# kluonj/HelFEM

Measured on AMD Instinct MI355X. Metric: scf_iteration_wall_time_fock_plus_geneig_nbf4230, lower is better.
Workload: dtype f64; 1 GPU; diatomic Z1=7 Z2=7 R=2.068 PBE, nelem=5 nnodes=15 nquad=75 lmmax=[20,20] (Nbf=4230, Nang=61, Nrad=70), XC grid 92x13, symmetry blocks [1380, 1470, 1380]: J+XC Fock build + eig_gsym_sub + density per step; parallelism=shard1, density=occupied orbitals of the core Hamiltonian

## Files before the change

helfem_amd/csrc/hip/common.h:

```cpp
#pragma once
#include <hip/hip_runtime.h>
#include <cstdint>
#include <cstring>
#include <map>
#include <stdexcept>
#include <string>
#include <vector>

#include "../../../include/helfem_gpu.h"
#include "../host/atomic_basis.h"
#include "../host/diatomic_basis.h"
#include "../host/tuning.h"

namespace hfg {
using helfem::TrdMode, helfem::tuning;

void set_error(const std::string &msg);

#define HFG_HIP_CHECK(expr)                                                                          \
  do {                                                                                               \
    hipError_t _e = (expr);                                                                          \
    if (_e != hipSuccess)                                                                            \
      throw std::runtime_error(std::string("HIP error: ") + hipGetErrorString(_e) + " in " + #expr + \
                               " (" + __FILE__ + ":" + std::to_string(__LINE__) + ")");              \
  } while (0)

template <typename T>
struct DevBuf {
  T *p = nullptr;
  size_t n = 0;
  DevBuf() {}
  DevBuf(const DevBuf &) = delete;
  DevBuf &operator=(const DevBuf &) = delete;
  ~DevBuf() { release(); }
  void release() {
    if (p) (void)hipFree(p);
    p = nullptr;
    n = 0;
  }
  void resize(size_t count) {
    if (count <= n) return;
    release();
    HFG_HIP_CHECK(hipMalloc((void **)&p, count * sizeof(T)));
    n = count;
  }
  void upload(const std::vector<T> &h, hipStream_t s) {
    resize(h.size() ? h.size() : 1);
    if (h.size()) HFG_HIP_CHECK(hipMemcpyAsync(p, h.data(), h.size() * sizeof(T), hipMemcpyHostToDevice, s));
  }
};

template <typename T>
bool upload_cached(DevBuf<T> &buf, std::vector<T> &cache, const std::vector<T> &h, hipStream_t s) {
  if (buf.p && cache.size() == h.size() && buf.n >= h.size() &&
      (h.empty() || memcmp((const void *)cache.data(), (const void *)h.data(), h.size() * sizeof(T)) == 0))
    return false;
  HFG_HIP_CHECK(hipStreamSynchronize(s));
  cache = h;
  buf.upload(cache, s);
  return true;
}

struct ProfEntry {
  double ms = 0.0;
  int64_t launches = 0;
  std::vector<std::pair<hipEvent_t, hipEvent_t> > pending;
};

}

struct hfg_dev_tables;

struct hfg_ctx {
  int device = 0;
  hipStream_t stream = nullptr;
  bool own_stream = false;
  hipStream_t side_stream = nullptr;
  hipEvent_t side_ev[2] = {nullptr, nullptr};
  hipStream_t side();
  bool avoid_side = false;
  void drop_side();
  int shard_rank = 0, shard_n = 1;
  const double *fixed_sinvh = nullptr;
  unsigned long fixed_gen = 0;
  void fix_sinvh(const double *p) {
    fixed_sinvh = p;
    fixed_gen++;
  }
  bool profiling = false;
  std::map<std::string, hfg::ProfEntry> prof;
  std::vector<hipEvent_t> event_pool;
  hfg::DevBuf<double> ws[8];
  hfg::DevBuf<double> hstage;
  double *pinned = nullptr;
  size_t pinned_bytes = 0;

  void *pinned_buf(size_t bytes);
  hipEvent_t get_event();
  void prof_begin(const char *name);
  void prof_end(const char *name);
  void prof_collect();
};

struct hfg_basis {
  int kind = 0;
  helfem::diatomic::TwoDBasis b;
  helfem::atomic::TwoDBasis ab;
  hfg_dev_tables *dev = nullptr;
  hfg_dev_tables *dev_rs = nullptr;
  int dev_device = -1;
  hfg::DevBuf<double> dev_tei;
  bool tei_on_device = false;

  size_t Nbf() const { return kind ? ab.Nbf() : b.Nbf(); }
  size_t Ndummy() const { return kind ? ab.Nbf() : b.Ndummy(); }
  size_t Nrad() const { return kind ? ab.Nrad() : b.Nrad(); }
  size_t Nang() const { return kind ? ab.Nang() : b.Nang(); }
  size_t Nel() const { return kind ? ab.Nel() : b.Nel(); }
  size_t max_Nprim() const { return kind ? ab.max_Nprim() : b.max_Nprim(); }
  bool have_tei() const { return tei_on_device || (kind ? ab.have_tei : b.have_tei); }
};

namespace hfg {
struct GemmTask {
  const double *A;
  const double *B;
  double *C;
  int M, N, K, lda, ldb, ldc;
  int tA = 0, tB = 0;
  double alpha = 1.0, beta = 0.0;
  int sym = 0;
  int over = 0;
};
static_assert(sizeof(GemmTask) == 80, "GemmTask is compared bytewise: keep it free of padding");

struct ProfScope {
  hfg_ctx *c;
  const char *n;
  ProfScope(hfg_ctx *ctx, const char *name) : c(ctx), n(name) {
    if (c->profiling) c->prof_begin(n);
  }
  ~ProfScope() {
    if (c->profiling) c->prof_end(n);
  }
};
}
```

helfem_amd/csrc/hip/dc.hip:

```cpp
#include "common.h"
#include <cstring>
#include "wave.h"

namespace hfg {

constexpr int DC_LEAF = 16;
constexpr int DC_MAXB = 8;
#define DC_EPS 2.220446049250313e-16

struct DCNode {
  int blk, lo, mid, hi;
};

struct DCBatch {
  int n[DC_MAXB];
  double *d[DC_MAXB];
  double *d2[DC_MAXB];
  double *e[DC_MAXB];
  double *Qa[DC_MAXB], *Qb[DC_MAXB];
  double *U[DC_MAXB], *Qg[DC_MAXB], *Qn[DC_MAXB];
  double *Ds[DC_MAXB], *zs[DC_MAXB], *dnd[DC_MAXB], *znd[DC_MAXB], *mu[DC_MAXB], *lam[DC_MAXB], *zhat[DC_MAXB];
  double *rotc[DC_MAXB], *rots[DC_MAXB];
  int *src[DC_MAXB], *flag[DC_MAXB], *nd[DC_MAXB], *org[DC_MAXB], *roti[DC_MAXB], *rotj[DC_MAXB], *rank[DC_MAXB];
  int *ndpos[DC_MAXB];
};

__global__ void k_dc_tear(DCBatch b, const DCNode *__restrict__ nodes, int nnodes, double *__restrict__ rho) {
  int i = blockIdx.x * blockDim.x + threadIdx.x;
  if (i >= nnodes) return;
  DCNode nd = nodes[i];
  double r = b.e[nd.blk][nd.mid - 1];
  rho[i] = r;
  b.d[nd.blk][nd.mid - 1] -= fabs(r);
  b.d[nd.blk][nd.mid] -= fabs(r);
}

__global__ __launch_bounds__(64) void k_dc_leaf(DCBatch b, const DCNode *__restrict__ leaves, int nleaves,
                                                int *__restrict__ status) {
  __shared__ double ds[DC_LEAF], es[DC_LEAF], zt[DC_LEAF][DC_LEAF + 1];
  int li = blockIdx.x;
  if (li >= nleaves) return;
  DCNode lf = leaves[li];
  const int lo = lf.lo, s = lf.hi - lf.lo;
  const int lane = threadIdx.x;
  const int ld = b.n[lf.blk];
  double *d = b.d[lf.blk], *e = b.e[lf.blk];
  if (lane < s) {
    ds[lane] = d[lo + lane];
    es[lane] = (lane < s - 1) ? e[lo + lane] : 0.0;
    for (int c = 0; c < s; c++) zt[c][lane] = (c == lane) ? 1.0 : 0.0;
  }
  __syncthreads();
  for (int l = 0; l < s; l++) {
    int iter = 0;
    int m;
    do {
      for (m = l; m + 1 < s; m++) {
        double dd = fabs(ds[m]) + fabs(ds[m + 1]);
        if (fabs(es[m]) <= DC_EPS * dd) break;
      }
      if (m != l) {
        if (iter++ == 300) {
          if (lane == 0) status[0] = 1;
          break;
        }
        double g = (ds[l + 1] - ds[l]) / (2.0 * es[l]);
        double r = hypot(g, 1.0);
        g = ds[m] - ds[l] + es[l] / (g + (g >= 0.0 ? fabs(r) : -fabs(r)));
        double sn = 1.0, c = 1.0, p = 0.0;
        bool under = false;
        for (int i = m - 1; i >= l; i--) {
          double f = sn * es[i], bb = c * es[i];
          r = hypot(f, g);
          __syncthreads();
          es[i + 1] = r;
          if (r == 0.0) {
            ds[i + 1] -= p;
            es[m] = 0.0;
            under = true;
            __syncthreads();
            break;
          }
          sn = f / r;
          c = g / r;
          g = ds[i + 1] - p;
          r = (ds[i] - g) * sn + 2.0 * c * bb;
          p = sn * r;
          __syncthreads();
          ds[i + 1] = g + p;
          g = c * r - bb;
          if (lane < s) {
            double fz = zt[i + 1][lane], zi = zt[i][lane];
            zt[i + 1][lane] = sn * zi + c * fz;
            zt[i][lane] = c * zi - sn * fz;
          }
          __syncthreads();
        }
        if (under) continue;
        __syncthreads();
        ds[l] -= p;
        es[l] = g;
        es[m] = 0.0;
        __syncthreads();
      }
    } while (m != l);
  }
  __syncthreads();
  if (lane < s) {
    double v = ds[lane];
    int rk = 0;
    for (int j = 0; j < s; j++) rk += (ds[j] < v) || (ds[j] == v && j < lane);
    d[lo + rk] = v;
    double *Q = b.Qa[lf.blk];
    for (int k = 0; k < s; k++) Q[(size_t)(lo + rk) * ld + lo + k] = zt[lane][k];
  }
}

constexpr int DC_SQZ = 20;
__global__ __launch_bounds__(256) void k_dc_prepare(DCBatch b, const DCNode *__restrict__ nodes,
                                                    const double *__restrict__ rho_all, int node0,
                                                    int *__restrict__ kcount, int *__restrict__ nrot,
                                                    double *__restrict__ rho_eff, GemmTask *__restrict__ tasks,
                                                    double *__restrict__ gscratch, size_t gstride) {
  extern __shared__ double lds_[];
  double *sh = gscratch ? gscratch + (size_t)blockIdx.x * gstride : lds_;
  const int ni = node0 + blockIdx.x;
  const DCNode nd = nodes[ni];
  const int blk = nd.blk, lo = nd.lo, mid = nd.mid, hi = nd.hi;
  const int n1 = mid - lo, n = hi - lo;
  const int ld = b.n[blk];
  double *sD = sh;
  double *sz = sh + n;
  int *ssrc = (int *)(sh + 2 * n);
  int *sflag = ssrc + n;
  int *snd = sflag + n;
  int *rm = snd + n;
  unsigned long long *rotw = (unsigned long long *)(rm + n);
  __shared__ int nrm_sh, candk_sh;
  __shared__ double red[8];
  __shared__ double tol_sh;
  __shared__ int k_sh;
  const double *d = b.d[blk];
  const double *Q = b.Qa[blk];
  const double rs = rho_all[ni];
  const double sgn = (rs >= 0.0) ? 1.0 : -1.0;
  const double rho = 2.0 * fabs(rs);
  const double isq2 = 0.7071067811865475244;

  double dmax = 0.0, zmax = 0.0;
  for (int j = threadIdx.x; j < n; j += blockDim.x) {
    double Dj = d[lo + j];
    double zj = (j < n1 ? Q[(size_t)(lo + j) * ld + (mid - 1)] : sgn * Q[(size_t)(lo + j) * ld + mid]) * isq2;
    int pos;
    if (j < n1) {
      int a = 0, c = n - n1;
      while (a < c) {
        int h = (a + c) >> 1;
        if (d[mid + h] < Dj) a = h + 1;
        else c = h;
      }
      pos = j + a;
    } else {
      int a = 0, c = n1;
      while (a < c) {
        int h = (a + c) >> 1;
        if (d[lo + h] <= Dj) a = h + 1;
        else c = h;
      }
      pos = (j - n1) + a;
    }
    sD[pos] = Dj;
    sz[pos] = zj;
    ssrc[pos] = j;
    dmax = fmax(dmax, fabs(Dj));
    zmax = fmax(zmax, fabs(zj));
  }
  double m2 = fmax(dmax, zmax);
  m2 = wave_max(m2);
  zmax = wave_max(zmax);
  if ((threadIdx.x & 63) == 0) {
    red[threadIdx.x >> 6] = m2;
    red[4 + (threadIdx.x >> 6)] = zmax;
  }
  __syncthreads();
  const double mm = fmax(fmax(red[0], red[1]), fmax(red[2], red[3]));
  const double zz = fmax(fmax(red[4], red[5]), fmax(red[6], red[7]));
  const double tol = 8.0 * DC_EPS * mm;
  __shared__ int scan[256];
  int fast = 0, fast_k = 0;
  if (!(rho * zz <= tol)) {
    const int tid = threadIdx.x;
    const int chunk = (n + 255) / 256, c0 = tid * chunk, c1 = min(n, c0 + chunk);
    int cnt = 0;
    for (int j = c0; j < c1; j++) {
      const int small = (rho * fabs(sz[j]) <= tol) ? 1 : 0;
      sflag[j] = small;
      cnt += 1 - small;
    }
    scan[tid] = cnt;
    __syncthreads();
    for (int off = 1; off < 256; off <<= 1) {
      const int v = (tid >= off) ? scan[tid - off] : 0;
      __syncthreads();
      scan[tid] += v;
      __syncthreads();
    }
    fast_k = scan[255];
    int r = scan[tid] - cnt;
    for (int j = c0; j < c1; j++)
      if (!sflag[j]) snd[r++] = j;
    __syncthreads();
    int rot = 0;
    for (int base = 0; base < fast_k; base += 256) {
      const int q = base + tid;
      int f = 0;
      if (q >= 1 && q < fast_k) {
        const int pj = snd[q - 1], j = snd[q];
        const double zj = sz[j], zp = sz[pj], t = sD[j] - sD[pj];
        f = (fabs(t * zj * zp) <= tol * (zj * zj + zp * zp)) ? 1 : 0;
      }
      const unsigned long long m = __ballot(f);
      if ((tid & 63) == 0) rotw[(base >> 6) + (tid >> 6)] = m;
      rot |= f;
    }
    fast = __syncthreads_or(rot) ? 0 : 1;
  }
  if (threadIdx.x == 0) {
    nrm_sh = 0;
    candk_sh = fast_k;
  }
  if (threadIdx.x == 0) {
    tol_sh = tol;
    int k = 0, nr = 0;
    int *ndl = snd;
    int *ri = b.roti[blk] + lo, *rj = b.rotj[blk] + lo;
    double *rc = b.rotc[blk] + lo, *rsn = b.rots[blk] + lo;
    if (rho * zz <= tol) {
      for (int j = 0; j < n; j++) sflag[j] = 1;
    } else if (fast) {
      k = fast_k;
    } else if (n <= 256 * DC_SQZ) {
      const int K = fast_k, nw = (K + 63) >> 6;
      int q = 1;
      while (q < K) {
        int wq = q >> 6;
        unsigned long long m = rotw[wq] & (~0ull << (q & 63));
        while (m == 0 && ++wq < nw) m = rotw[wq];
        if (m == 0) break;
        q = (wq << 6) + __ffsll((long long)m) - 1;
        if (q >= K) break;
        int pq = q - 1, pj = snd[pq];
        double zp = sz[pj], dp = sD[pj];
        while (q < K) {
          const int j = snd[q];
          const double zj = sz[j], dj = sD[j], t = dj - dp;
          if (!(fabs(t * zj * zp) <= tol * (zj * zj + zp * zp))) {
            q++;
            break;
          }
          const double tau = hypot(zj, zp);
          const double c = zj / tau, sn = -zp / tau;
          sz[j] = tau;
          sz[pj] = 0.0;
          ri[nr] = pj;
          rj[nr] = j;
          rc[nr] = c;
          rsn[nr] = sn;
          rm[nr] = pq;
          nr++;
          const double tt = dp * c * c + dj * sn * sn;
          const double dn = dp * sn * sn + dj * c * c;
          sD[j] = dn;
          sD[pj] = tt;
          sflag[pj] = 1;
          pj = j;
          pq = q;
          zp = tau;
          dp = dn;
          q++;
        }
      }
      k = K - nr;
      nrm_sh = nr;
    } else {
      int pj = -1;
      double zp = 0.0, dp = 0.0;
      for (int j = 0; j < n; j++) {
        const double zj = sz[j], dj = sD[j];
        if (rho * fabs(zj) <= tol) {
          sflag[j] = 1;
          continue;
        }
        sflag[j] = 0;
        if (pj < 0) {
          pj = j;
          zp = zj;
          dp = dj;
          continue;
        }
        const double t = dj - dp;
        if (fabs(t * zj * zp) <= tol * (zj * zj + zp * zp)) {
          const double tau = hypot(zj, zp);
          const double c = zj / tau, s = -zp / tau;
          sz[j] = tau;
          sz[pj] = 0.0;
          ri[nr] = pj;
          rj[nr] = j;
          rc[nr] = c;
          rsn[nr] = s;
          nr++;
          const double tt = dp * c * c + dj * s * s;
          const double dn = dp * s * s + dj * c * c;
          sD[j] = dn;
          sD[pj] = tt;
          sflag[pj] = 1;
          pj = j;
          zp = tau;
          dp = dn;
        } else {
          ndl[k++] = pj;
          pj = j;
          zp = zj;
          dp = dj;
        }
      }
      if (pj >= 0) ndl[k++] = pj;
    }
    k_sh = k;
    kcount[ni] = k;
    nrot[ni] = nr;
    rho_eff[ni] = rho;
    GemmTask t;
    t.A = b.Qg[blk] + (size_t)lo * ld + lo;
    t.B = b.U[blk] + (size_t)lo * ld + lo;
    t.C = b.Qn[blk] + (size_t)lo * ld + lo;
    t.M = n;
    t.N = k;
    t.K = k;
    t.lda = t.ldb = t.ldc = ld;
    tasks[blockIdx.x] = t;
  }
  __syncthreads();
  if (nrm_sh > 0) {
    const int K = candk_sh, nrm = nrm_sh;
    const int chunk = (K + 255) / 256, c0 = threadIdx.x * chunk;
    int vals[DC_SQZ], newi[DC_SQZ];
#pragma unroll
    for (int e = 0; e < DC_SQZ; e++) {
      const int q = c0 + e;
      newi[e] = -1;
      vals[e] = 0;
      if (e < chunk && q < K) {
        int a = 0, c = nrm;
        while (a < c) {
          const int h = (a + c) >> 1;
          if (rm[h] < q) a = h + 1;
          else c = h;
        }
        if (!(a < nrm && rm[a] == q)) {
          newi[e] = q - a;
          vals[e] = snd[q];
        }
      }
    }
    __syncthreads();
#pragma unroll
    for (int e = 0; e < DC_SQZ; e++)
      if (newi[e] >= 0) snd[newi[e]] = vals[e];
    __syncthreads();
  }
  const int k = k_sh;
  for (int j = threadIdx.x; j < n; j += blockDim.x) {
    b.Ds[blk][lo + j] = sD[j];
    b.zs[blk][lo + j] = sz[j];
    b.src[blk][lo + j] = ssrc[j];
    b.flag[blk][lo + j] = sflag[j];
  }
  for (int c = threadIdx.x; c < k; c += blockDim.x) {
    int sidx = snd[c];
    b.ndpos[blk][lo + sidx] = c;
    b.nd[blk][lo + c] = sidx;
    b.dnd[blk][lo + c] = sD[sidx];
    b.znd[blk][lo + c] = sz[sidx];
  }
}

__global__ __launch_bounds__(256) void k_dc_rotate(DCBatch b, const DCNode *__restrict__ nodes, int node0,
                                                   const int *__restrict__ nrot) {
  const int ni = node0 + blockIdx.y;
  const DCNode nd = nodes[ni];
  const int nr = nrot[ni];
  if (nr == 0) return;
  const int lo = nd.lo, n = nd.hi - nd.lo, blk = nd.blk;
  const int ld = b.n[blk];
  const int r = blockIdx.x * blockDim.x + threadIdx.x;
  __shared__ int scp[256], scj[256];
  __shared__ double sc[256], ss[256];
  const int *src = b.src[blk] + lo;
  double *Q = b.Qa[blk] + lo + r;
  for (int t0 = 0; t0 < nr; t0 += 256) {
    const int t = t0 + threadIdx.x;
    if (t < nr) {
      scp[threadIdx.x] = lo + src[b.roti[blk][lo + t]];
      scj[threadIdx.x] = lo + src[b.rotj[blk][lo + t]];
      sc[threadIdx.x] = b.rotc[blk][lo + t];
      ss[threadIdx.x] = b.rots[blk][lo + t];
    }
    __syncthreads();
    if (r < n) {
      const int cnt = min(256, nr - t0);
      for (int u = 0; u < cnt; u++) {
        const int cp = scp[u], cj = scj[u];
        const double c = sc[u], s = ss[u];
        const double qp = Q[(size_t)cp * ld], qj = Q[(size_t)cj * ld];
        Q[(size_t)cp * ld] = c * qp + s * qj;
        Q[(size_t)cj * ld] = -s * qp + c * qj;
      }
    }
    __syncthreads();
  }
}


__global__ __launch_bounds__(256) void k_dc_secular(DCBatch b, const DCNode *__restrict__ nodes, int node0,
                                                    const int *__restrict__ kcount,
                                                    const double *__restrict__ rho_eff) {
  const int ni = node0 + blockIdx.y;
  const int k = kcount[ni];
  const int i = blockIdx.x * 4 + (threadIdx.x >> 6);
  if (i >= k) return;
  const int lane = threadIdx.x & 63;
  const DCNode nd = nodes[ni];
  const int blk = nd.blk, lo = nd.lo;
  const double *d = b.dnd[blk] + lo, *z = b.znd[blk] + lo;
  const double rho = rho_eff[ni];
  int org;
  double lob, hib, y;
  if (i < k - 1) {
    double gap = d[i + 1] - d[i];
    double midp = 0.5 * gap;
    double di = d[i];
    double s = 0.0;
    for (int j = lane; j < k; j += 64) s += z[j] * z[j] / ((d[j] - di) - midp);
    double fm = 1.0 + rho * wave_sum(s);
    if (fm > 0.0) {
      org = i;
      lob = 0.0;
      hib = midp;
    } else {
      org = i + 1;
      lob = -midp;
      hib = 0.0;
    }
  } else {
    org = k - 1;
    double s = 0.0;
    for (int j = lane; j < k; j += 64) s += z[j] * z[j];
    lob = 0.0;
    hib = rho * wave_sum(s);
  }
  const double dorg = d[org];
  y = 0.5 * (lob + hib);
  for (int it = 0; it < 100; it++) {
    double psi = 0.0, phi = 0.0, dpsi = 0.0, dphi = 0.0;
    for (int j = lane; j < k; j += 64) {
      double D = (d[j] - dorg) - y;
      double t = z[j] * z[j] / D;
      if (j <= i) {
        psi += t;
        dpsi += t / D;
      } else {
        phi += t;
        dphi += t / D;
      }
    }
    psi = rho * wave_sum(psi);
    phi = rho * wave_sum(phi);
    dpsi = rho * wave_sum(dpsi);
    dphi = rho * wave_sum(dphi);
    double w = 1.0 + psi + phi;
    double err = 16.0 * DC_EPS * (1.0 + fabs(psi) + fabs(phi)) + DC_EPS * fabs(y) * (dpsi + dphi);
    if (fabs(w) <= err) break;
    if (w < 0.0) lob = y;
    else hib = y;
    double eta;
    if (i < k - 1) {
      double Di = (d[i] - dorg) - y, Dq = (d[i + 1] - dorg) - y;
      double c = w - Di * dpsi - Dq * dphi;
      double a = (Di + Dq) * w - Di * Dq * (dpsi + dphi);
      double bb = Di * Dq * w;
      if (c == 0.0) eta = (a != 0.0) ? bb / a : 0.0;
      else {
        double disc = a * a - 4.0 * bb * c;
        disc = sqrt(fmax(disc, 0.0));
        eta = (a <= 0.0) ? (a - disc) / (2.0 * c) : 2.0 * bb / (a + disc);
      }
    } else {
      double Di = -y;
      double c = w - Di * dpsi;
      double S = Di * Di * dpsi;
      eta = (c != 0.0) ? Di + S / c : 0.0;
    }
    double yn = y + eta;
    if (!(yn > lob && yn < hib)) yn = 0.5 * (lob + hib);
    bool done = (yn == y) || (hib - lob <= 2.0 * DC_EPS * fmax(fabs(lob), fabs(hib)));
    y = yn;
    if (done) break;
  }
  if (lane == 0) {
    b.org[blk][lo + i] = org;
    b.mu[blk][lo + i] = y;
    b.lam[blk][lo + i] = dorg + y;
  }
}

__global__ __launch_bounds__(256) void k_dc_zhat(DCBatch b, const DCNode *__restrict__ nodes, int node0,
                                                 const int *__restrict__ kcount, const double *__restrict__ rho_eff) {
  const int ni = node0 + blockIdx.y;
  const int k = kcount[ni];
  const int j = blockIdx.x * 4 + (threadIdx.x >> 6);
  if (j >= k) return;
  const int lane = threadIdx.x & 63;
  const DCNode nd = nodes[ni];
  const int blk = nd.blk, lo = nd.lo;
  const double *d = b.dnd[blk] + lo, *mu = b.mu[blk] + lo;
  const int *org = b.org[blk] + lo;
  const double dj = d[j];
  double prod = 1.0;
  for (int i = lane; i < k; i += 64) {
    double num = (d[org[i]] - dj) + mu[i];
    prod *= (i == j) ? num : num / (d[i] - dj);
  }
  prod = wave_prod(prod);
  if (lane == 0) {
    double zh = sqrt(fabs(prod) / rho_eff[ni]);
    b.zhat[blk][lo + j] = (b.znd[blk][lo + j] >= 0.0) ? zh : -zh;
  }
}

__global__ __launch_bounds__(256) void k_dc_U(DCBatch b, const DCNode *__restrict__ nodes, int node0,
                                              const int *__restrict__ kcount) {
  const int ni = node0 + blockIdx.y;
  const int k = kcount[ni];
  const int i = blockIdx.x * 4 + (threadIdx.x >> 6);
  if (i >= k) return;
  const int lane = threadIdx.x & 63;
  const DCNode nd = nodes[ni];
  const int blk = nd.blk, lo = nd.lo;
  const int ld = b.n[blk];
  const double *d = b.dnd[blk] + lo, *zh = b.zhat[blk] + lo;
  const double dorg = d[b.org[blk][lo + i]], mui = b.mu[blk][lo + i];
  double s = 0.0;
  for (int j = lane; j < k; j += 64) {
    double v = zh[j] / ((d[j] - dorg) - mui);
    s += v * v;
  }
  s = 1.0 / sqrt(wave_sum(s));
  double *Ucol = b.U[blk] + (size_t)(lo + i) * ld + lo;
  for (int j = lane; j < k; j += 64) Ucol[j] = zh[j] / ((d[j] - dorg) - mui) * s;
}

__global__ void k_dc_gather(DCBatch b, const DCNode *__restrict__ nodes, int node0,
                            const int *__restrict__ kcount) {
  const int ni = node0 + blockIdx.z;
  const int k = kcount[ni];
  const int c = blockIdx.y;
  if (c >= k) return;
  const DCNode nd = nodes[ni];
  const int blk = nd.blk, lo = nd.lo, n = nd.hi - nd.lo;
  const int ld = b.n[blk];
  int r = blockIdx.x * blockDim.x + threadIdx.x;
  if (r >= n) return;
  const double *Q = b.Qa[blk];
  int sidx = b.nd[blk][lo + c];
  int col = lo + b.src[blk][lo + sidx];
  b.Qg[blk][(size_t)(lo + c) * ld + lo + r] = Q[(size_t)col * ld + lo + r];
}

__global__ __launch_bounds__(256) void k_dc_rank(DCBatch b, const DCNode *__restrict__ nodes, int node0,
                                                 const int *__restrict__ kcount) {
  extern __shared__ double sh[];
  const int ni = node0 + blockIdx.x;
  const DCNode nd = nodes[ni];
  const int blk = nd.blk, lo = nd.lo, n = nd.hi - nd.lo;
  if ((int)blockIdx.y * 32 >= n) return;
  const int *flag = b.flag[blk] + lo;
  for (int s = threadIdx.x; s < n; s += blockDim.x) {
    sh[s] = flag[s] ? b.Ds[blk][lo + s] : b.lam[blk][lo + b.ndpos[blk][lo + s]];
  }
  __syncthreads();
  const int s = blockIdx.y * 32 + (threadIdx.x >> 3), part = threadIdx.x & 7;
  const int per = (n + 7) >> 3, j0 = part * per, j1 = min(n, j0 + per);
  const bool ok = s < n;
  const double v = ok ? sh[s] : 0.0;
  int rk = 0;
  if (ok) {
    int j = j0;
    for (; j + 8 <= j1; j += 8) {
#pragma unroll
      for (int u = 0; u < 8; u++) {
        const double x = sh[j + u];
        rk += (x < v) || (x == v && j + u < s);
      }
    }
    for (; j < j1; j++) {
      const double x = sh[j];
      rk += (x < v) || (x == v && j < s);
    }
  }
  rk += __builtin_amdgcn_update_dpp(0, rk, 0xb1, 0xf, 0xf, true);
  rk += __builtin_amdgcn_update_dpp(0, rk, 0x4e, 0xf, 0xf, true);
  rk += __builtin_amdgcn_update_dpp(0, rk, 0x141, 0xf, 0xf, true);
  if (ok && part == 0) {
    b.rank[blk][lo + s] = rk;
    b.d2[blk][lo + rk] = v;
  }
}

__global__ void k_dc_scatter(DCBatch b, const DCNode *__restrict__ nodes, int node0, const int *__restrict__ kcount) {
  const int ni = node0 + blockIdx.z;
  const DCNode nd = nodes[ni];
  const int blk = nd.blk, lo = nd.lo, n = nd.hi - nd.lo;
  const int s = blockIdx.y;
  if (s >= n) return;
  int r = blockIdx.x * blockDim.x + threadIdx.x;
  if (r >= n) return;
  const int ld = b.n[blk];
  const int k = kcount[ni];
  const double *Q = b.Qa[blk];
  int rk = b.rank[blk][lo + s];
  double v;
  if (b.flag[blk][lo + s]) {
    v = Q[(size_t)(lo + b.src[blk][lo + s]) * ld + lo + r];
  } else {
    const int *ndl = b.nd[blk] + lo;
    int a = 0, c = k;
    while (a < c) {
      int h = (a + c) >> 1;
      if (ndl[h] < s) a = h + 1;
      else c = h;
    }
    v = b.Qn[blk][(size_t)(lo + a) * ld + lo + r];
  }
  b.Qb[blk][(size_t)(lo + rk) * ld + lo + r] = v;
}

__global__ void k_dc_copyback(DCBatch b, const DCNode *__restrict__ nodes, int node0) {
  const int ni = node0 + blockIdx.z;
  const DCNode nd = nodes[ni];
  const int blk = nd.blk, lo = nd.lo, n = nd.hi - nd.lo;
  const int c = blockIdx.y;
  if (c >= n) return;
  int r = blockIdx.x * blockDim.x + threadIdx.x;
  if (r >= n) return;
  const int ld = b.n[blk];
  b.Qa[blk][(size_t)(lo + c) * ld + lo + r] = b.Qb[blk][(size_t)(lo + c) * ld + lo + r];
  if (c == 0) b.d[blk][lo + r] = b.d2[blk][lo + r];
}

void gemm_tasklist64_dev(hfg_ctx *ctx, const GemmTask *dtasks, int ntasks, int maxM, int maxN);
typedef double double4_t __attribute__((ext_vector_type(4)));

__global__ __launch_bounds__(256) void k_dgemm_tasks(const GemmTask *__restrict__ tasks) {
  constexpr int BM = 64, BN = 64, BK = 16, PAD = 16;
  __shared__ double As[BK][BM + PAD];
  __shared__ double Bs[BK][BN + PAD];
  const GemmTask t = tasks[blockIdx.y];
  const int M = t.M, N = t.N, K = t.K;
  if (M <= 0 || N <= 0) return;
  const int nbm = (M + BM - 1) / BM, nbn = (N + BN - 1) / BN;
  if ((int)blockIdx.x >= nbm * nbn) return;
  const int bm = (blockIdx.x % nbm) * BM, bn = (blockIdx.x / nbm) * BN;
  const int tid = threadIdx.x, wave = tid >> 6, lane = tid & 63;
  const int wm = (wave & 1) * 32, wn = (wave >> 1) * 32;
  const int l15 = lane & 15, l4 = lane >> 4;
  double4_t acc[2][2];
  for (int i = 0; i < 2; i++)
    for (int j = 0; j < 2; j++) acc[i][j] = (double4_t){0.0, 0.0, 0.0, 0.0};
  for (int k0 = 0; k0 < K; k0 += BK) {
    __syncthreads();
#pragma unroll
    for (int r = 0; r < 4; r++) {
      int e = tid + 256 * r;
      int m = e % BM, kk = e / BM;
      int gm = bm + m, gk = k0 + kk;
      As[kk][m] = (gm < M && gk < K) ? t.A[(size_t)gk * t.lda + gm] : 0.0;
      int k2 = e % BK, n2 = e / BK;
      int gn = bn + n2, gk2 = k0 + k2;
      Bs[k2][n2] = (gn < N && gk2 < K) ? t.B[(size_t)gn * t.ldb + gk2] : 0.0;
    }
    __syncthreads();
#pragma unroll
    for (int kk = 0; kk < BK; kk += 4) {
      double fa[2], fb[2];
      for (int i = 0; i < 2; i++) fa[i] = As[kk + l4][wm + i * 16 + l15];
      for (int j = 0; j < 2; j++) fb[j] = Bs[kk + l4][wn + j * 16 + l15];
      for (int i = 0; i < 2; i++)
        for (int j = 0; j < 2; j++) acc[i][j] = __builtin_amdgcn_mfma_f64_16x16x4f64(fb[j], fa[i], acc[i][j], 0, 0, 0);
    }
  }
  for (int i = 0; i < 2; i++)
    for (int j = 0; j < 2; j++)
      for (int r = 0; r < 4; r++) {
        int gm = bm + wm + i * 16 + l15, gn = bn + wn + j * 16 + l4 + 4 * r;
        if (gm < M && gn < N) t.C[(size_t)gn * t.ldc + gm] = acc[i][j][r];
      }
}

void gemm_tasks_dev(hfg_ctx *ctx, const GemmTask *dtasks, int ntasks, int max_tiles) {
  if (ntasks <= 0 || max_tiles <= 0) return;
  for (int t0 = 0; t0 < ntasks; t0 += 65535) {
    int nt = std::min(65535, ntasks - t0);
    hipLaunchKernelGGL(k_dgemm_tasks, dim3(max_tiles, nt), dim3(256), 0, ctx->stream, dtasks + t0);
  }
  HFG_HIP_CHECK(hipGetLastError());
}

struct DCWork {
  DevBuf<double> prep_scratch;
  DevBuf<double> d2[DC_MAXB], Qb[DC_MAXB], U[DC_MAXB], Qg[DC_MAXB], Qn[DC_MAXB];
  DevBuf<double> vec[DC_MAXB];
  DevBuf<int> ivec[DC_MAXB];
  DevBuf<DCNode> nodes;
  DevBuf<double> rho, rho_eff;
  DevBuf<int> kcount, nrot, status;
  DevBuf<GemmTask> tasks;
  std::vector<int> key;
  std::vector<DCNode> hnodes;
  std::vector<int> level_off;
  std::vector<int> level_maxn;
  int nleaves = 0;
};
static std::map<hfg_ctx *, DCWork *> g_dc;
void dc_release(hfg_ctx *ctx) {
  auto it = g_dc.find(ctx);
  if (it != g_dc.end()) {
    delete it->second;
    g_dc.erase(it);
  }
}

static int build_tree(int blk, int lo, int hi, std::vector<std::vector<DCNode> > &byheight) {
  DCNode nd;
  nd.blk = blk;
  nd.lo = lo;
  nd.hi = hi;
  if (hi - lo <= DC_LEAF) {
    nd.mid = lo;
    if (byheight.empty()) byheight.resize(1);
    byheight[0].push_back(nd);
    return 0;
  }
  int mid = lo + (hi - lo) / 2;
  nd.mid = mid;
  int h = 1 + std::max(build_tree(blk, lo, mid, byheight), build_tree(blk, mid, hi, byheight));
  if ((int)byheight.size() <= h) byheight.resize(h + 1);
  byheight[h].push_back(nd);
  return h;
}

void tridiag_dc_batch(hfg_ctx *ctx, int nblk, const int *ns, double *const *d, double *const *e, double *const *Z) {
  if (nblk > DC_MAXB) throw std::logic_error("tridiag_dc_batch: too many blocks");
  DCWork *wp;
  auto it = g_dc.find(ctx);
  if (it == g_dc.end()) {
    wp = new DCWork();
    g_dc[ctx] = wp;
  } else
    wp = it->second;
  DCWork &w = *wp;
  hipStream_t s = ctx->stream;
  std::vector<int> key(ns, ns + nblk);
  if (key != w.key) {
    std::vector<std::vector<DCNode> > byh;
    for (int b = 0; b < nblk; b++) build_tree(b, 0, ns[b], byh);
    w.hnodes.clear();
    w.level_off.clear();
    w.level_maxn.clear();
    w.hnodes.insert(w.hnodes.end(), byh[0].begin(), byh[0].end());
    w.nleaves = (int)byh[0].size();
    for (size_t h = 1; h < byh.size(); h++) {
      w.level_off.push_back((int)w.hnodes.size());
      int mx = 0;
      for (auto &nd : byh[h]) mx = std::max(mx, nd.hi - nd.lo);
      w.level_maxn.push_back(mx);
      w.hnodes.insert(w.hnodes.end(), byh[h].begin(), byh[h].end());
    }
    w.level_off.push_back((int)w.hnodes.size());
    w.nodes.resize(w.hnodes.size());
    HFG_HIP_CHECK(hipMemcpyAsync(w.nodes.p, w.hnodes.data(), sizeof(DCNode) * w.hnodes.size(), hipMemcpyHostToDevice, s));
    HFG_HIP_CHECK(hipStreamSynchronize(s));
    w.key = key;
    w.rho.resize(w.hnodes.size());
    w.rho_eff.resize(w.hnodes.size());
    w.kcount.resize(w.hnodes.size());
    w.nrot.resize(w.hnodes.size());
    w.tasks.resize(w.hnodes.size());
    w.status.resize(4);
  }
  DCBatch b;
  int nmax = 0;
  for (int i = 0; i < nblk; i++) {
    int n = ns[i];
    nmax = std::max(nmax, n);
    size_t nn = (size_t)n * n;
    w.d2[i].resize(n);
    w.Qb[i].resize(nn);
    w.U[i].resize(nn);
    w.Qg[i].resize(nn);
    w.Qn[i].resize(nn);
    w.vec[i].resize((size_t)9 * n);
    w.ivec[i].resize((size_t)8 * n);
    b.n[i] = n;
    b.d[i] = d[i];
    b.d2[i] = w.d2[i].p;
    b.e[i] = e[i];
    b.Qa[i] = Z[i];
    b.Qb[i] = w.Qb[i].p;
    b.U[i] = w.U[i].p;
    b.Qg[i] = w.Qg[i].p;
    b.Qn[i] = w.Qn[i].p;
    double *v = w.vec[i].p;
    b.Ds[i] = v;
    b.zs[i] = v + n;
    b.dnd[i] = v + 2 * n;
    b.znd[i] = v + 3 * n;
    b.mu[i] = v + 4 * n;
    b.lam[i] = v + 5 * n;
    b.zhat[i] = v + 6 * n;
    b.rotc[i] = v + 7 * n;
    b.rots[i] = v + 8 * n;
    int *iv = w.ivec[i].p;
    b.src[i] = iv;
    b.flag[i] = iv + n;
    b.nd[i] = iv + 2 * n;
    b.org[i] = iv + 3 * n;
    b.roti[i] = iv + 4 * n;
    b.rotj[i] = iv + 5 * n;
    b.rank[i] = iv + 6 * n;
    b.ndpos[i] = iv + 7 * n;
    HFG_HIP_CHECK(hipMemsetAsync(Z[i], 0, sizeof(double) * nn, s));
  }
  HFG_HIP_CHECK(hipMemsetAsync(w.status.p, 0, sizeof(int) * 4, s));
  const int ninternal = (int)w.hnodes.size() - w.nleaves;
  if (ninternal > 0)
    hipLaunchKernelGGL(k_dc_tear, dim3((ninternal + 255) / 256), dim3(256), 0, s, b, w.nodes.p + w.nleaves, ninternal,
                       w.rho.p + w.nleaves);
  hipLaunchKernelGGL(k_dc_leaf, dim3(w.nleaves), dim3(64), 0, s, b, w.nodes.p, w.nleaves, w.status.p);
  const int nlevels = (int)w.level_off.size() - 1;
  for (int h = 0; h < nlevels; h++) {
    const int node0 = w.level_off[h], nn = w.level_off[h + 1] - node0;
    const int mx = w.level_maxn[h];
    size_t shb = (size_t)mx * (2 * sizeof(double) + 4 * sizeof(int)) + ((size_t)mx / 64 + 2) * sizeof(unsigned long long);
    double *gscr = nullptr;
    size_t gstride = 0;
    if (shb > 150 * 1024) {
      gstride = (shb + 7) / 8 + 8;
      w.prep_scratch.resize(gstride * nn);
      gscr = w.prep_scratch.p;
      shb = 0;
    } else if (shb > 64 * 1024)
      HFG_HIP_CHECK(hipFuncSetAttribute((const void *)k_dc_prepare, hipFuncAttributeMaxDynamicSharedMemorySize, (int)shb));
    hipLaunchKernelGGL(k_dc_prepare, dim3(nn), dim3(256), shb, s, b, w.nodes.p, w.rho.p, node0, w.kcount.p, w.nrot.p,
                       w.rho_eff.p, w.tasks.p, gscr, gstride);
    hipLaunchKernelGGL(k_dc_rotate, dim3((mx + 255) / 256, nn), dim3(256), 0, s, b, w.nodes.p, node0, w.nrot.p);
    hipLaunchKernelGGL(k_dc_secular, dim3((mx + 3) / 4, nn), dim3(256), 0, s, b, w.nodes.p, node0, w.kcount.p,
                       w.rho_eff.p);
    hipLaunchKernelGGL(k_dc_zhat, dim3((mx + 3) / 4, nn), dim3(256), 0, s, b, w.nodes.p, node0, w.kcount.p, w.rho_eff.p);
    hipLaunchKernelGGL(k_dc_U, dim3((mx + 3) / 4, nn), dim3(256), 0, s, b, w.nodes.p, node0, w.kcount.p);
    hipLaunchKernelGGL(k_dc_gather, dim3((mx + 255) / 256, mx, nn), dim3(256), 0, s, b, w.nodes.p, node0, w.kcount.p);
    if (tuning().dc_gemm_small) {
      int tiles = ((mx + 63) / 64) * ((mx + 63) / 64);
      hipLaunchKernelGGL(k_dgemm_tasks, dim3(tiles, nn), dim3(256), 0, s, w.tasks.p);
    } else
      gemm_tasklist64_dev(ctx, w.tasks.p, nn, mx, mx);
    size_t shr = (size_t)mx * sizeof(double);
    if (shr > 64 * 1024)
      HFG_HIP_CHECK(hipFuncSetAttribute((const void *)k_dc_rank, hipFuncAttributeMaxDynamicSharedMemorySize, (int)shr));
    hipLaunchKernelGGL(k_dc_rank, dim3(nn, (mx + 31) / 32), dim3(256), shr, s, b, w.nodes.p, node0, w.kcount.p);
    hipLaunchKernelGGL(k_dc_scatter, dim3((mx + 255) / 256, mx, nn), dim3(256), 0, s, b, w.nodes.p, node0, w.kcount.p);
    hipLaunchKernelGGL(k_dc_copyback, dim3((mx + 255) / 256, mx, nn), dim3(256), 0, s, b, w.nodes.p, node0);
  }
  HFG_HIP_CHECK(hipGetLastError());
  if (tuning().dc_dbg) {
    std::vector<int> hk(w.hnodes.size()), hr(w.hnodes.size());
    HFG_HIP_CHECK(hipMemcpyAsync(hk.data(), w.kcount.p, sizeof(int) * hk.size(), hipMemcpyDeviceToHost, s));
    HFG_HIP_CHECK(hipMemcpyAsync(hr.data(), w.nrot.p, sizeof(int) * hr.size(), hipMemcpyDeviceToHost, s));
    HFG_HIP_CHECK(hipStreamSynchronize(s));
    for (int h = std::max(0, nlevels - 3); h < nlevels; h++)
      for (int q = w.level_off[h]; q < w.level_off[h + 1]; q++)
        fprintf(stderr, "dc level %d node %d: n %d, roots %d, rotations %d\n", h, q, w.hnodes[q].hi - w.hnodes[q].lo, hk[q], hr[q]);
  }
}

int dc_status(hfg_ctx *ctx) {
  auto it = g_dc.find(ctx);
  if (it == g_dc.end()) return 0;
  int st = 0;
  HFG_HIP_CHECK(hipMemcpyAsync(&st, it->second->status.p, sizeof(int), hipMemcpyDeviceToHost, ctx->stream));
  HFG_HIP_CHECK(hipStreamSynchronize(ctx->stream));
  return st;
}

}
```

helfem_amd/csrc/hip/eig.hip:

```cpp
#include "common.h"
#include "wave.h"
#include <cstdlib>
#include <cstring>

namespace hfg {

void gemm_tasklist_dev(hfg_ctx *ctx, const GemmTask *dtasks, int ntasks, int maxM, int maxN);
void gemm_tasklist_rect_dev(hfg_ctx *ctx, const GemmTask *dtasks, int ntasks, int maxM, int maxN);
void gemm_tasklist_split2_dev(hfg_ctx *ctx, const GemmTask *dtasks, int ntasks, int maxM, int maxN);
void gemm_tasklist64_dev(hfg_ctx *ctx, const GemmTask *dtasks, int ntasks, int maxM, int maxN);
bool gemm_prefers_128(hfg_ctx *ctx, long tiles128);
bool tridiagonalize_takes_chain(int nblk, const int *ns);
void gemm_tasklist_acc_dev(hfg_ctx *ctx, const GemmTask *dtasks, int ntasks, int maxM, int maxN, bool tile64);
void gemm_mirror_lower_dev(hfg_ctx *ctx, const GemmTask *dtasks, int ntasks, int maxN);
void gemm_dev(hfg_ctx *ctx, bool tA, bool tB, int M, int N, int K, double alpha, const double *A, int lda,
              const double *B, int ldb, double beta, double *C, int ldc);

void tridiag_dc_batch(hfg_ctx *ctx, int nblk, const int *ns, double *const *d, double *const *e, double *const *Z);
int dc_status(hfg_ctx *ctx);
void tridiagonalize_batch(hfg_ctx *ctx, int nblk, const int *ns, double *const *A, double *const *d, double *const *e,
                          double *const *tau);

constexpr int MAXB = 8;
struct EigBatch {
  int nblk;
  int n[MAXB];
  double *A[MAXB];
  double *d[MAXB];
  double *e[MAXB];
  double *tau[MAXB];
  double *v[MAXB];
  double *pp[MAXB];
  double *dots[MAXB];
  double *Z[MAXB];
  double *rot[MAXB];
  int *sweeps[MAXB];
  long rotcap[MAXB];
};

constexpr int TRD_NCS = 8;

__global__ void k_gather_block(const double *__restrict__ F, const double *__restrict__ S, int N,
                               const int64_t *__restrict__ rows, const int64_t *__restrict__ cols, int n,
                               double *__restrict__ Fb, double *__restrict__ Xb) {
  int i = blockIdx.x * blockDim.x + threadIdx.x;
  int j = blockIdx.y;
  if (i >= n) return;
  Fb[(size_t)j * n + i] = F[(size_t)rows[j] * N + rows[i]];
  Xb[(size_t)j * n + i] = S[(size_t)cols[j] * N + rows[i]];
}

__global__ void k_col_support(const double *__restrict__ S, int N, const int64_t *__restrict__ rows, int n,
                              int *__restrict__ flag) {
  int c = blockIdx.x;
  int any = 0;
  for (int i = threadIdx.x; i < n; i += blockDim.x)
    if (S[(size_t)c * N + rows[i]] != 0.0) any = 1;
  any = __syncthreads_or(any);
  if (threadIdx.x == 0) flag[c] = any;
}

__device__ inline void householder_of_column(const double *__restrict__ A, int n, int k, double *vsh, double *red,
                                             double &tau, double &beta) {
  const int m = n - k - 1;
  const double *x = A + (size_t)k * n + k + 1;
  double s = 0.0;
  for (int i = 1 + threadIdx.x; i < m; i += blockDim.x) s += x[i] * x[i];
  s = wave_sum(s);
  int nwave = blockDim.x / 64;
  if ((threadIdx.x & 63) == 0) red[threadIdx.x >> 6] = s;
  __syncthreads();
  double xn2 = 0.0;
  for (int w = 0; w < nwave; w++) xn2 += red[w];
  double alpha = x[0];
  double scale;
  if (xn2 == 0.0) {
    tau = 0.0;
    beta = alpha;
    scale = 0.0;
  } else {
    double nrm = sqrt(alpha * alpha + xn2);
    beta = (alpha >= 0.0) ? -nrm : nrm;
    tau = (beta - alpha) / beta;
    scale = 1.0 / (alpha - beta);
  }
  for (int i = threadIdx.x; i < m; i += blockDim.x) vsh[i] = (i == 0) ? 1.0 : x[i] * scale;
  __syncthreads();
}

__global__ __launch_bounds__(256) void k_trd_gemv(EigBatch b, int k) {
  extern __shared__ double sh[];
  const int blk = blockIdx.y;
  const int n = b.n[blk];
  if (k > n - 3) return;
  const int m = n - k - 1;
  const int nrs = (m + 63) / 64;
  const int rs = blockIdx.x / TRD_NCS, cs = blockIdx.x % TRD_NCS;
  if (rs >= nrs) return;
  double *A = b.A[blk];
  double *vsh = sh;
  double *red = sh + n;
  double tau, beta;
  householder_of_column(A, n, k, vsh, red, tau, beta);
  if (blockIdx.x == 0) {
    for (int i = threadIdx.x; i < m; i += blockDim.x) b.v[blk][i] = vsh[i];
    if (threadIdx.x == 0) {
      b.tau[blk][k] = tau;
      b.e[blk][k] = beta;
      b.d[blk][k] = A[(size_t)k * n + k];
    }
  }
  const int cchunk = (m + TRD_NCS - 1) / TRD_NCS;
  const int c0 = cs * cchunk, c1 = min(m, c0 + cchunk);
  const int wave = threadIdx.x >> 6, lane = threadIdx.x & 63;
  const int row = rs * 64 + lane;
  double acc = 0.0;
  if (row < m) {
    const double *a = A + (size_t)(k + 1) * n + (k + 1) + row;
    for (int c = c0 + wave; c < c1; c += 4) acc += a[(size_t)c * n] * vsh[c];
  }
  __syncthreads();
  red[wave * 64 + lane] = acc;
  __syncthreads();
  if (wave == 0) {
    double p = red[lane] + red[64 + lane] + red[128 + lane] + red[192 + lane];
    if (row < m) b.pp[blk][(size_t)cs * n + row] = p;
    double dv = (row < m) ? p * vsh[row] : 0.0;
    dv = wave_sum(dv);
    if (lane == 0) b.dots[blk][blockIdx.x] = dv;
  }
}

__global__ __launch_bounds__(256) void k_trd_update(EigBatch b, int k) {
  __shared__ double vr[64], vc[64], wr[64], wc[64];
  __shared__ double Ksh;
  const int blk = blockIdx.y;
  const int n = b.n[blk];
  if (k > n - 3) return;
  const int m = n - k - 1;
  const int nt = (m + 63) / 64;
  if ((int)blockIdx.x >= nt * nt) return;
  const int tr = blockIdx.x % nt, tc = blockIdx.x / nt;
  double *A = b.A[blk];
  const double tau = b.tau[blk][k];
  if (threadIdx.x == 0) {
    const int nrs = (m + 63) / 64;
    double s = 0.0;
    for (int i = 0; i < nrs * TRD_NCS; i++) s += b.dots[blk][i];
    Ksh = 0.5 * tau * tau * s;
  }
  __syncthreads();
  if (threadIdx.x < 128) {
    int which = threadIdx.x >> 6, l = threadIdx.x & 63;
    int idx = (which ? tc : tr) * 64 + l;
    double v = 0.0, w = 0.0;
    if (idx < m) {
      v = b.v[blk][idx];
      double p = 0.0;
      for (int cs = 0; cs < TRD_NCS; cs++) p += b.pp[blk][(size_t)cs * n + idx];
      w = tau * p - Ksh * v;
    }
    if (which) {
      vc[l] = v;
      wc[l] = w;
    } else {
      vr[l] = v;
      wr[l] = w;
    }
  }
  __syncthreads();
  const int lane = threadIdx.x & 63, wave = threadIdx.x >> 6;
  const int row = tr * 64 + lane;
  if (row < m) {
    double *a = A + (size_t)(k + 1) * n + (k + 1) + row;
    for (int c = wave; c < 64; c += 4) {
      int col = tc * 64 + c;
      if (col < m) a[(size_t)col * n] -= vr[lane] * wc[c] + wr[lane] * vc[c];
    }
  }
  if (blockIdx.x == 0) {
    for (int i = 1 + threadIdx.x; i < m; i += blockDim.x) A[(size_t)k * n + k + 1 + i] = b.v[blk][i];
  }
}

__global__ void k_trd_finish(EigBatch b) {
  int blk = blockIdx.x;
  if (threadIdx.x != 0) return;
  int n = b.n[blk];
  double *A = b.A[blk];
  if (n >= 2) {
    b.d[blk][n - 2] = A[(size_t)(n - 2) * n + (n - 2)];
    b.e[blk][n - 2] = A[(size_t)(n - 2) * n + (n - 1)];
    b.tau[blk][n - 2] = 0.0;
  }
  b.d[blk][n - 1] = A[(size_t)(n - 1) * n + (n - 1)];
  b.e[blk][n - 1] = 0.0;
}

__global__ void k_tql_values(EigBatch b) {
  int blk = blockIdx.x;
  if (threadIdx.x != 0) return;
  const int n = b.n[blk];
  double *d = b.d[blk], *e = b.e[blk];
  double *rot = b.rot[blk];
  int *sw = b.sweeps[blk];
  long nrot = 0;
  int nsw = 0;
  int status = 0;
  const long cap = b.rotcap[blk];
  for (int l = 0; l < n && !status; l++) {
    int iter = 0;
    int m;
    do {
      for (m = l; m + 1 < n; m++) {
        double dd = fabs(d[m]) + fabs(d[m + 1]);
        if (fabs(e[m]) <= 2.220446049250313e-16 * dd) break;
      }
      if (m != l) {
        if (iter++ == 300) {
          status = 1;
          break;
        }
        if (nrot + (m - l) > cap || 4 * (nsw + 1) + 2 >= 4 * 64 * n) {
          status = 2;
          break;
        }
        double g = (d[l + 1] - d[l]) / (2.0 * e[l]);
        double r = hypot(g, 1.0);
        g = d[m] - d[l] + e[l] / (g + (g >= 0.0 ? fabs(r) : -fabs(r)));
        double s = 1.0, c = 1.0, p = 0.0;
        int cnt = 0;
        bool under = false;
        int i;
        for (i = m - 1; i >= l; i--) {
          double f = s * e[i], bb = c * e[i];
          r = hypot(f, g);
          e[i + 1] = r;
          if (r == 0.0) {
            d[i + 1] -= p;
            e[m] = 0.0;
            under = true;
            break;
          }
          s = f / r;
          c = g / r;
          g = d[i + 1] - p;
          r = (d[i] - g) * s + 2.0 * c * bb;
          p = s * r;
          d[i + 1] = g + p;
          g = c * r - bb;
          rot[2 * (nrot + cnt)] = c;
          rot[2 * (nrot + cnt) + 1] = s;
          cnt++;
        }
        sw[2 + 4 * nsw + 0] = l;
        sw[2 + 4 * nsw + 1] = m;
        sw[2 + 4 * nsw + 2] = (int)(nrot & 0x7fffffff);
        sw[2 + 4 * nsw + 3] = cnt;
        nsw++;
        nrot += cnt;
        if (under) continue;
        d[l] -= p;
        e[l] = g;
        e[m] = 0.0;
      }
    } while (m != l);
  }
  sw[0] = nsw;
  sw[1] = status;
}

__global__ void k_set_identity(EigBatch b) {
  int blk = blockIdx.z;
  int n = b.n[blk];
  int i = blockIdx.x * blockDim.x + threadIdx.x, j = blockIdx.y;
  if (i < n && j < n) b.Z[blk][(size_t)j * n + i] = (i == j) ? 1.0 : 0.0;
}

__global__ void k_tql_apply(EigBatch b) {
  int blk = blockIdx.y;
  int n = b.n[blk];
  int k = blockIdx.x * blockDim.x + threadIdx.x;
  if (k >= n) return;
  double *Z = b.Z[blk] + k;
  const double *rot = b.rot[blk];
  const int *sw = b.sweeps[blk];
  int nsw = sw[0];
  long off = 0;
  for (int q = 0; q < nsw; q++) {
    int m = sw[2 + 4 * q + 1], cnt = sw[2 + 4 * q + 3];
    double hi = Z[(size_t)m * n];
    int i = m - 1;
    for (int t = 0; t < cnt; t++, i--) {
      double c = rot[2 * (off + t)], s = rot[2 * (off + t) + 1];
      double lo = Z[(size_t)i * n];
      Z[(size_t)(i + 1) * n] = s * lo + c * hi;
      hi = c * lo - s * hi;
    }
    Z[(size_t)(i + 1) * n] = hi;
    off += cnt;
  }
}

template <int NR>
__global__ __launch_bounds__(256) void k_backtransform(EigBatch b) {
  int blk = blockIdx.y;
  int n = b.n[blk];
  int col = blockIdx.x * 4 + (threadIdx.x >> 6);
  int lane = threadIdx.x & 63;
  if (col >= n) return;
  const double *A = b.A[blk];
  const double *tau = b.tau[blk];
  double *z = b.Z[blk] + (size_t)col * n;
  double zr[NR];
#pragma unroll
  for (int r = 0; r < NR; r++) {
    int i = lane + 64 * r;
    zr[r] = (i < n) ? z[i] : 0.0;
  }
  for (int k = n - 3; k >= 0; k--) {
    double t = tau[k];
    if (t == 0.0) continue;
    const double *v = A + (size_t)k * n;
    double s = 0.0;
    double vr[NR];
#pragma unroll
    for (int r = 0; r < NR; r++) {
      int i = lane + 64 * r;
      double vi = 0.0;
      if (i == k + 1) vi = 1.0;
      else if (i > k + 1 && i < n) vi = v[i];
      vr[r] = vi;
      s += vi * zr[r];
    }
    s = wave_sum(s);
    s *= t;
#pragma unroll
    for (int r = 0; r < NR; r++) zr[r] -= s * vr[r];
  }
#pragma unroll
  for (int r = 0; r < NR; r++) {
    int i = lane + 64 * r;
    if (i < n) z[i] = zr[r];
  }
}

__global__ __launch_bounds__(256) void k_backtransform_lds(EigBatch b) {
  extern __shared__ double sh[];
  int blk = blockIdx.y;
  int n = b.n[blk];
  int wave = threadIdx.x >> 6, lane = threadIdx.x & 63;
  int col = blockIdx.x * 4 + wave;
  if (col >= n) return;
  const double *A = b.A[blk];
  const double *tau = b.tau[blk];
  double *z = b.Z[blk] + (size_t)col * n;
  double *zs = sh + (size_t)wave * n;
  for (int i = lane; i < n; i += 64) zs[i] = z[i];
  for (int k = n - 3; k >= 0; k--) {
    double t = tau[k];
    if (t == 0.0) continue;
    const double *v = A + (size_t)k * n;
    double s = 0.0;
    for (int i = k + 1 + lane; i < n; i += 64) s += ((i == k + 1) ? 1.0 : v[i]) * zs[i];
    s = wave_sum(s);
    s *= t;
    for (int i = k + 1 + lane; i < n; i += 64) zs[i] -= s * ((i == k + 1) ? 1.0 : v[i]);
  }
  for (int i = lane; i < n; i += 64) z[i] = zs[i];
}

constexpr int RANK_SEG = 8;
__global__ __launch_bounds__(256) void k_rank(const double *__restrict__ E, int n, int *__restrict__ rank) {
  __shared__ double sE[256];
  const int i = blockIdx.x * 256 + threadIdx.x;
  const double ei = (i < n) ? E[i] : 0.0;
  const int seg = (n + RANK_SEG - 1) / RANK_SEG;
  const int j0 = blockIdx.y * seg, j1 = min(n, j0 + seg);
  int r = 0;
  for (int c = j0; c < j1; c += 256) {
    __syncthreads();
    sE[threadIdx.x] = (c + (int)threadIdx.x < j1) ? E[c + threadIdx.x] : 0.0;
    __syncthreads();
    const int m = min(256, j1 - c);
    if (m == 256) {
#pragma unroll 16
      for (int jj = 0; jj < 256; jj++) {
        const double ej = sE[jj];
        r += (ej < ei) || (ej == ei && c + jj < i);
      }
    } else {
      for (int jj = 0; jj < m; jj++) {
        const double ej = sE[jj];
        r += (ej < ei) || (ej == ei && c + jj < i);
      }
    }
  }
  if (i < n && r) atomicAdd(&rank[i], r);
}
static void launch_rank(hfg_ctx *ctx, const double *E, int n, int *rank) {
  HFG_HIP_CHECK(hipMemsetAsync(rank, 0, sizeof(int) * n, ctx->stream));
  hipLaunchKernelGGL(k_rank, dim3((n + 255) / 256, RANK_SEG), dim3(256), 0, ctx->stream, E, n, rank);
}

__global__ void k_scatter_cols(const double *__restrict__ Cb, int nrow, int ncol, const int64_t *__restrict__ rows,
                               const int *__restrict__ rank, int coff, const double *__restrict__ Eb, int ldc,
                               double *__restrict__ Cout, double *__restrict__ Eout) {
  int i = blockIdx.x * blockDim.x + threadIdx.x;
  int j = blockIdx.y;
  if (i >= nrow) return;
  int c = rank[coff + j];
  size_t r = rows ? (size_t)rows[i] : (size_t)i;
  Cout[(size_t)c * ldc + r] = Cb[(size_t)j * nrow + i];
  if (i == 0) Eout[c] = Eb[j];
}

constexpr int BT_KB = 64;

__global__ void k_bt_extract(EigBatch b, double *const *__restrict__ Vx) {
  const int blk = blockIdx.z;
  const int n = b.n[blk];
  const int j = blockIdx.y;
  const int g = blockIdx.x * blockDim.x + threadIdx.x;
  if (j >= n || g >= n) return;
  double v = 0.0;
  if (j <= n - 3) {
    if (g == j + 1) v = 1.0;
    else if (g > j + 1) v = b.A[blk][(size_t)j * n + g];
  }
  Vx[blk][(size_t)j * n + g] = v;
}

constexpr int BT_PW = 2 * BT_KB;
constexpr int BT_WREP = 4;
__global__ __launch_bounds__(256) void k_bt_wpair(EigBatch b, double *const *__restrict__ Wpart, double *const *__restrict__ W,
                                                  double *const *__restrict__ Cc, int S, int GS, int npair, int pair,
                                                  int mirror) {
  __shared__ double sC[BT_KB][BT_KB + 1];
  __shared__ double s1[4][BT_KB];
  const int blk = blockIdx.y;
  const int n = b.n[blk];
  const int j0 = pair * BT_PW;
  if (j0 > n - 3) return;
  const int kb1 = min(BT_KB, n - 2 - (j0 + BT_KB));
  const int tid = threadIdx.x, cl = tid >> 6, i = tid & 63;
  if (kb1 > 0) {
    constexpr int NE = BT_KB * BT_KB / 256;
    double c[NE];
#pragma unroll
    for (int u = 0; u < NE; u++) c[u] = 0.0;
    for (int sl = 0; sl < GS; sl++) {
      const double *src = Cc[blk] + ((size_t)sl * npair + pair) * BT_KB * BT_KB + tid;
#pragma unroll
      for (int u = 0; u < NE; u++) c[u] += src[256 * u];
    }
#pragma unroll
    for (int u = 0; u < NE; u++) {
      const int t = tid + 256 * u;
      sC[t % BT_KB][t / BT_KB] = c[u];
    }
  }
  const size_t tot = (size_t)BT_PW * n;
  double a0[BT_WREP], a1[BT_WREP];
#pragma unroll
  for (int rep = 0; rep < BT_WREP; rep++) {
    const int col = (blockIdx.x * BT_WREP + rep) * 4 + cl;
    a0[rep] = 0.0;
    a1[rep] = 0.0;
    if (col < n) {
      for (int sl = 0; sl < S; sl++) {
        a0[rep] += Wpart[blk][(size_t)sl * tot + (size_t)col * BT_PW + i];
        a1[rep] += Wpart[blk][(size_t)sl * tot + (size_t)col * BT_PW + BT_KB + i];
      }
    }
  }
  if (mirror) {
    const int kb0 = min(BT_KB, n - 2 - j0);
#pragma unroll
    for (int rep = 0; rep < BT_WREP; rep++) {
      const int col = (blockIdx.x * BT_WREP + rep) * 4 + cl;
      __syncthreads();
      s1[cl][i] = (i < kb0) ? a0[rep] : 0.0;
      __syncthreads();
      if (col < n) {
        double r1 = 0.0;
        if (kb1 > 0 && i < kb1) {
          double corr = 0.0;
          for (int j = 0; j < kb0; j++) corr += sC[j][i] * s1[cl][j];
          r1 = a1[rep] - corr;
        }
        W[blk][(size_t)col * BT_PW + i] = a0[rep];
        W[blk][(size_t)col * BT_PW + BT_KB + i] = r1;
      }
    }
    return;
  }
#pragma unroll
  for (int rep = 0; rep < BT_WREP; rep++) {
    const int col = (blockIdx.x * BT_WREP + rep) * 4 + cl;
    __syncthreads();
    s1[cl][i] = (kb1 > 0 && i < kb1) ? a1[rep] : 0.0;
    __syncthreads();
    if (col < n) {
      double r0 = a0[rep];
      if (kb1 > 0) {
        double corr = 0.0;
        for (int j = 0; j < kb1; j++) corr += sC[i][j] * s1[cl][j];
        r0 -= corr;
      }
      W[blk][(size_t)col * BT_PW + i] = r0;
      W[blk][(size_t)col * BT_PW + BT_KB + i] = (kb1 > 0 && i < kb1) ? a1[rep] : 0.0;
    }
  }
}

constexpr int BT_GS = 4;
__global__ __launch_bounds__(64) void k_bt_T(EigBatch b, double *const *__restrict__ G, double *const *__restrict__ T,
                                             int P) {
  __shared__ double sT[BT_KB][BT_KB + 1];
  __shared__ double sG[BT_KB][BT_KB + 1];
  __shared__ double sg[BT_KB];
  const int blk = blockIdx.y, p = blockIdx.x;
  const int n = b.n[blk];
  const int j0 = p * BT_KB;
  if (j0 > n - 3) return;
  const int kb = min(BT_KB, n - 2 - j0);
  double *Tp = T[blk] + (size_t)p * BT_KB * BT_KB;
  const int t = threadIdx.x;
  for (int c0 = 0; c0 < BT_KB; c0 += 16) {
    double g[16];
#pragma unroll
    for (int u = 0; u < 16; u++) g[u] = 0.0;
#pragma unroll
    for (int sl = 0; sl < BT_GS; sl++) {
      const double *src = G[blk] + ((size_t)sl * P + p) * BT_KB * BT_KB + (size_t)c0 * BT_KB + t;
#pragma unroll
      for (int u = 0; u < 16; u++) g[u] += src[(size_t)u * BT_KB];
    }
#pragma unroll
    for (int u = 0; u < 16; u++) {
      sG[c0 + u][t] = g[u];
      sT[t][c0 + u] = 0.0;
    }
  }
  __shared__ double stau[BT_KB];
  stau[t] = (t < kb) ? b.tau[blk][j0 + t] : 0.0;
  __syncthreads();
  for (int i = 0; i < kb; i++) {
    const double ti = stau[i];
    sg[t] = (t < i) ? sG[i][t] : 0.0;
    __syncthreads();
    if (t < i) {
      double acc0 = 0.0, acc1 = 0.0, acc2 = 0.0, acc3 = 0.0;
#pragma unroll
      for (int k = 0; k < BT_KB; k += 4) {
        acc0 += sT[t][k] * sg[k];
        acc1 += sT[t][k + 1] * sg[k + 1];
        acc2 += sT[t][k + 2] * sg[k + 2];
        acc3 += sT[t][k + 3] * sg[k + 3];
      }
      sT[t][i] = -ti * ((acc0 + acc1) + (acc2 + acc3));
    }
    if (t == i) sT[i][i] = ti;
    __syncthreads();
  }
  for (int c = 0; c < BT_KB; c++) Tp[(size_t)c * BT_KB + t] = sT[t][c];
}

struct EigWork {
  bool split_full = false;
  bool tile64 = false;
  std::vector<int64_t> asm_rows;
  DevBuf<long long> asm_rows_dev;
  bool folded = false;
  DevBuf<double> Y[MAXB];
  DevBuf<GemmTask> btslabR, btupdR;
  std::vector<GemmTask> h_btslabR, h_btupdR;
  DevBuf<double> A[MAXB], d[MAXB], e[MAXB], tau[MAXB], v[MAXB], pp[MAXB], dots[MAXB], Z[MAXB], rot[MAXB];
  DevBuf<int> sweeps[MAXB];
  DevBuf<int> ibuf1, ibuf2;
  DevBuf<GemmTask> gtasks, bttasks, btslab, btgram, btcpl, btupd;
  std::vector<GemmTask> h_gtasks, h_bttasks, h_btslab, h_btgram, h_btcpl, h_btupd;
  std::vector<double *> h_btptr;
  DevBuf<double> Vx[MAXB], G[MAXB], T[MAXB], VT[MAXB], Wb[MAXB], Wp[MAXB], Cc[MAXB];
  DevBuf<double *> btptr;
  bool used_dc = true;
  DevBuf<double> idx;
  const double *sup_S = nullptr;
  unsigned long sup_gen = 0;
  int sup_N = 0;
  std::vector<int64_t> sup_ptr, sup_idx;
};
static std::map<hfg_ctx *, EigWork *> g_work;
static EigWork &work_for(hfg_ctx *ctx) {
  auto it = g_work.find(ctx);
  if (it != g_work.end()) return *it->second;
  EigWork *w = new EigWork();
  g_work[ctx] = w;
  return *w;
}
void eig_release(hfg_ctx *ctx) {
  auto it = g_work.find(ctx);
  if (it != g_work.end()) {
    delete it->second;
    g_work.erase(it);
  }
}

struct CopySlices {
  const double *src[16];
  double *dst[16];
  int n[16];
};
__global__ void k_copy_slices(CopySlices c) {
  const int q = blockIdx.y;
  for (int i = blockIdx.x * blockDim.x + threadIdx.x; i < c.n[q]; i += gridDim.x * blockDim.x) c.dst[q][i] = c.src[q][i];
}
static void copy_slices(hipStream_t s, const std::vector<const double *> &src, const std::vector<double *> &dst, const std::vector<int> &n) {
  for (size_t q0 = 0; q0 < src.size(); q0 += 16) {
    CopySlices c{};
    const int m = (int)std::min<size_t>(16, src.size() - q0);
    int nmax = 0;
    for (int q = 0; q < m; q++) {
      c.src[q] = src[q0 + q];
      c.dst[q] = dst[q0 + q];
      c.n[q] = n[q0 + q];
      nmax = std::max(nmax, n[q0 + q]);
    }
    if (nmax > 0) hipLaunchKernelGGL(k_copy_slices, dim3((nmax + 255) / 256, m), dim3(256), 0, s, c);
  }
}

struct TrPtrs {
  const double *src[MAXB];
  double *dst[MAXB];
  int n[MAXB];
};
__global__ __launch_bounds__(256) void k_transpose_batch(TrPtrs t) {
  __shared__ double tile[64][65];
  const int blk = blockIdx.z, n = t.n[blk];
  const int bi = blockIdx.x * 64, bj = blockIdx.y * 64;
  if (bi >= n || bj >= n) return;
  const int tx = threadIdx.x & 63, ty = threadIdx.x >> 6;
  for (int c = ty; c < 64; c += 4) {
    const int gm = bi + tx, gn = bj + c;
    tile[c][tx] = (gm < n && gn < n) ? t.src[blk][(size_t)gn * n + gm] : 0.0;
  }
  __syncthreads();
  for (int c = ty; c < 64; c += 4) {
    const int gm = bj + tx, gn = bi + c;
    if (gm < n && gn < n) t.dst[blk][(size_t)gn * n + gm] = tile[tx][c];
  }
}

static void bt_wy_setup(hfg_ctx *ctx, EigWork &w, const EigBatch &b, int nblk, const int *ns, int nmax, bool fold = false) {
  hipStream_t s = ctx->stream;
  const int P = (nmax - 3) / BT_KB + 1;
  const int NP = (P + 1) / 2;
  constexpr int BT_S = 6;
  std::vector<double *> ptrs(6 * (size_t)nblk);
  for (int k = 0; k < nblk; k++) {
    const int n = ns[k];
    w.Vx[k].resize((size_t)n * n);
    w.G[k].resize((size_t)BT_GS * P * BT_KB * BT_KB);
    w.T[k].resize((size_t)P * BT_KB * BT_KB);
    w.VT[k].resize((size_t)n * P * BT_KB);
    w.Wb[k].resize((size_t)BT_PW * n);
    w.Wp[k].resize((size_t)BT_S * BT_PW * n);
    w.Cc[k].resize((size_t)BT_GS * NP * BT_KB * BT_KB);
    ptrs[k] = w.Vx[k].p;
    ptrs[nblk + k] = w.G[k].p;
    ptrs[2 * nblk + k] = w.T[k].p;
    ptrs[3 * nblk + k] = w.Wp[k].p;
    ptrs[4 * nblk + k] = w.Wb[k].p;
    ptrs[5 * nblk + k] = w.Cc[k].p;
  }
  upload_cached(w.btptr, w.h_btptr, ptrs, s);
  GemmTask none;
  none.A = none.B = nullptr;
  none.C = nullptr;
  none.M = none.N = none.K = 0;
  none.lda = none.ldb = none.ldc = 1;
  auto kb_of = [&](int k, int p) { return std::max(0, std::min(BT_KB, ns[k] - 2 - p * BT_KB)); };
  auto chunk_of = [](int len, int parts) { return ((len + parts - 1) / parts + 15) / 16 * 16; };

  std::vector<GemmTask> gram((size_t)BT_GS * P * nblk, none), vt((size_t)P * nblk, none);
  for (int p = 0; p < P; p++)
    for (int k = 0; k < nblk; k++) {
      const int n = ns[k], j0 = p * BT_KB, kb = kb_of(k, p);
      if (kb <= 0) continue;
      const int r0 = j0 + 1, mr = n - r0;
      const double *Vp = w.Vx[k].p + (size_t)j0 * n + r0;
      const int chunk = chunk_of(mr, BT_GS);
      for (int sl = 0; sl < BT_GS; sl++) {
        GemmTask g = none;
        const int k0 = sl * chunk, kk = std::max(0, std::min(chunk, mr - k0));
        g.A = g.B = Vp + (kk > 0 ? k0 : 0);
        g.C = w.G[k].p + ((size_t)sl * P + p) * BT_KB * BT_KB;
        g.tA = 1;
        g.M = g.N = kb;
        g.K = kk;
        g.lda = g.ldb = n;
        g.ldc = BT_KB;
        gram[((size_t)sl * P + p) * nblk + k] = g;
      }
      const int rp = (p & ~1) * BT_KB + 1;
      GemmTask g = none;
      g.A = w.Vx[k].p + (size_t)j0 * n + rp;
      g.B = w.T[k].p + (size_t)p * BT_KB * BT_KB;
      g.C = w.VT[k].p + (size_t)j0 * n + rp;
      g.M = n - rp;
      g.N = g.K = kb;
      g.lda = n;
      g.ldb = BT_KB;
      g.ldc = n;
      vt[(size_t)p * nblk + k] = g;
    }
  upload_cached(w.btgram, w.h_btgram, gram, s);
  upload_cached(w.bttasks, w.h_bttasks, vt, s);

  std::vector<GemmTask> cpl((size_t)BT_GS * NP * nblk, none), slab((size_t)NP * BT_S * nblk, none), upd((size_t)NP * nblk, none);
  for (int g2 = 0; g2 < NP; g2++)
    for (int k = 0; k < nblk; k++) {
      const int n = ns[k], p0 = 2 * g2, j0 = p0 * BT_KB;
      const int kb0 = kb_of(k, p0), kb1 = (p0 + 1 < P) ? kb_of(k, p0 + 1) : 0;
      if (kb0 <= 0) continue;
      const int r0 = j0 + 1, mr = n - r0, kbp = kb0 + kb1;
      if (kb1 > 0) {
        const int r1 = j0 + BT_KB + 1, m1 = n - r1;
        const int chunk = chunk_of(m1, BT_GS);
        for (int sl = 0; sl < BT_GS; sl++) {
          GemmTask c = none;
          const int k0 = sl * chunk, kk = std::max(0, std::min(chunk, m1 - k0));
          c.A = w.Vx[k].p + (size_t)j0 * n + r1 + (kk > 0 ? k0 : 0);
          c.B = w.VT[k].p + (size_t)(j0 + BT_KB) * n + r1 + (kk > 0 ? k0 : 0);
          c.C = w.Cc[k].p + ((size_t)sl * NP + g2) * BT_KB * BT_KB;
          c.tA = 1;
          c.M = kb0;
          c.N = kb1;
          c.K = kk;
          c.lda = c.ldb = n;
          c.ldc = BT_KB;
          cpl[((size_t)sl * NP + g2) * nblk + k] = c;
        }
      }
      const int chunk = chunk_of(mr, BT_S);
      for (int sl = 0; sl < BT_S; sl++) {
        GemmTask q = none;
        const int k0 = sl * chunk, kk = std::max(0, std::min(chunk, mr - k0));
        q.A = w.Vx[k].p + (size_t)j0 * n + r0 + (kk > 0 ? k0 : 0);
        q.B = b.Z[k] + r0 + (kk > 0 ? k0 : 0);
        q.C = w.Wp[k].p + (size_t)sl * BT_PW * n;
        q.tA = 1;
        q.M = kbp;
        q.N = n;
        q.K = kk;
        q.lda = q.ldb = n;
        q.ldc = BT_PW;
        slab[((size_t)g2 * BT_S + sl) * nblk + k] = q;
      }
      GemmTask u = none;
      u.A = w.VT[k].p + (size_t)j0 * n + r0;
      u.B = w.Wb[k].p;
      u.C = b.Z[k] + r0;
      u.M = mr;
      u.N = n;
      u.K = kbp;
      u.lda = n;
      u.ldb = BT_PW;
      u.ldc = n;
      u.alpha = -1.0;
      u.beta = 1.0;
      upd[(size_t)g2 * nblk + k] = u;
    }
  upload_cached(w.btcpl, w.h_btcpl, cpl, s);
  upload_cached(w.btslab, w.h_btslab, slab, s);
  upload_cached(w.btupd, w.h_btupd, upd, s);
  if (fold) {
    std::vector<GemmTask> slabR((size_t)NP * BT_S * nblk, none), updR((size_t)NP * nblk, none);
    for (int g2 = 0; g2 < NP; g2++)
      for (int k = 0; k < nblk; k++) {
        const int n = ns[k], p0 = 2 * g2, j0 = p0 * BT_KB;
        const int kb0 = kb_of(k, p0), kb1 = (p0 + 1 < P) ? kb_of(k, p0 + 1) : 0;
        if (kb0 <= 0) continue;
        const int r0 = j0 + 1, mr = n - r0, kbp = kb0 + kb1;
        const int chunk = chunk_of(mr, BT_S);
        for (int sl = 0; sl < BT_S; sl++) {
          GemmTask q = none;
          const int k0 = sl * chunk, kk = std::max(0, std::min(chunk, mr - k0));
          q.A = w.VT[k].p + (size_t)j0 * n + r0 + (kk > 0 ? k0 : 0);
          q.B = w.Y[k].p + r0 + (kk > 0 ? k0 : 0);
          q.C = w.Wp[k].p + (size_t)sl * BT_PW * n;
          q.tA = 1;
          q.M = kbp;
          q.N = n;
          q.K = kk;
          q.lda = q.ldb = n;
          q.ldc = BT_PW;
          slabR[((size_t)g2 * BT_S + sl) * nblk + k] = q;
        }
        GemmTask u = none;
        u.A = w.Vx[k].p + (size_t)j0 * n + r0;
        u.B = w.Wb[k].p;
        u.C = w.Y[k].p + r0;
        u.M = mr;
        u.N = n;
        u.K = kbp;
        u.lda = n;
        u.ldb = BT_PW;
        u.ldc = n;
        u.alpha = -1.0;
        u.beta = 1.0;
        updR[(size_t)g2 * nblk + k] = u;
      }
    upload_cached(w.btslabR, w.h_btslabR, slabR, s);
    upload_cached(w.btupdR, w.h_btupdR, updR, s);
  }
}

static void bt_wy_prepare(hfg_ctx *ctx, EigWork &w, const EigBatch &b, int nblk, int nmax, bool on_side = false) {
  const int P = (nmax - 3) / BT_KB + 1;
  const bool use_side = (tuning().bt_side && !ctx->avoid_side) || on_side;
  hipStream_t main = ctx->stream, q = main;
  const bool prof = ctx->profiling;
  if (use_side) {
    q = ctx->side();
    HFG_HIP_CHECK(hipEventRecord(ctx->side_ev[0], main));
    HFG_HIP_CHECK(hipStreamWaitEvent(q, ctx->side_ev[0], 0));
    ctx->profiling = false;
    ctx->stream = q;
  }
  try {
    double *const *dptr = w.btptr.p;
    hipLaunchKernelGGL(k_bt_extract, dim3((nmax + 255) / 256, nmax, nblk), dim3(256), 0, q, b, dptr);
    gemm_tasklist64_dev(ctx, w.btgram.p, BT_GS * P * nblk, BT_KB, BT_KB);
    hipLaunchKernelGGL(k_bt_T, dim3(P, nblk), dim3(BT_KB), 0, q, b, dptr + nblk, dptr + 2 * nblk, P);
    gemm_tasklist64_dev(ctx, w.bttasks.p, P * nblk, nmax, BT_KB);
    gemm_tasklist64_dev(ctx, w.btcpl.p, BT_GS * ((P + 1) / 2) * nblk, BT_KB, BT_KB);
  } catch (...) {
    ctx->stream = main;
    ctx->profiling = prof;
    throw;
  }
  ctx->stream = main;
  ctx->profiling = prof;
  if (use_side) HFG_HIP_CHECK(hipEventRecord(ctx->side_ev[1], q));
}

static void bt_wy_apply(hfg_ctx *ctx, EigWork &w, const EigBatch &b, int nblk, int nmax) {
  hipStream_t s = ctx->stream;
  const int P = (nmax - 3) / BT_KB + 1, NP = (P + 1) / 2;
  constexpr int BT_S = 6;
  double *const *dptr = w.btptr.p;
  if (tuning().bt_side && !ctx->avoid_side) HFG_HIP_CHECK(hipStreamWaitEvent(s, ctx->side_ev[1], 0));
  for (int g = NP - 1; g >= 0; g--) {
    gemm_tasklist64_dev(ctx, w.btslab.p + (size_t)g * BT_S * nblk, BT_S * nblk, BT_PW, nmax);
    hipLaunchKernelGGL(k_bt_wpair, dim3((nmax + 4 * BT_WREP - 1) / (4 * BT_WREP), nblk), dim3(256), 0, s, b, dptr + 3 * nblk, dptr + 4 * nblk,
                       dptr + 5 * nblk, BT_S, BT_GS, NP, g, 0);
    gemm_tasklist_acc_dev(ctx, w.btupd.p + (size_t)g * nblk, nblk, nmax, nmax, tuning().acc_tile != 128);
  }
  HFG_HIP_CHECK(hipGetLastError());
}

static void bt_wy_fold_x(hfg_ctx *ctx, EigWork &w, const EigBatch &b, int nblk, const int *ns, int nmax, const double *const *X) {
  const int P = (nmax - 3) / BT_KB + 1, NP = (P + 1) / 2;
  constexpr int BT_S = 6;
  hipStream_t main = ctx->stream, q = ctx->side();
  const bool prof = ctx->profiling;
  ctx->profiling = false;
  ctx->stream = q;
  try {
    TrPtrs t;
    for (int k = 0; k < MAXB; k++) {
      t.src[k] = k < nblk ? X[k] : nullptr;
      t.dst[k] = k < nblk ? w.Y[k].p : nullptr;
      t.n[k] = k < nblk ? ns[k] : 0;
    }
    hipLaunchKernelGGL(k_transpose_batch, dim3((nmax + 63) / 64, (nmax + 63) / 64, nblk), dim3(256), 0, q, t);
    double *const *dptr = w.btptr.p;
    for (int g = 0; g < NP; g++) {
      gemm_tasklist64_dev(ctx, w.btslabR.p + (size_t)g * BT_S * nblk, BT_S * nblk, BT_PW, nmax);
      hipLaunchKernelGGL(k_bt_wpair, dim3((nmax + 4 * BT_WREP - 1) / (4 * BT_WREP), nblk), dim3(256), 0, q, b, dptr + 3 * nblk, dptr + 4 * nblk,
                         dptr + 5 * nblk, BT_S, BT_GS, NP, g, 1);
      gemm_tasklist_acc_dev(ctx, w.btupdR.p + (size_t)g * nblk, nblk, nmax, nmax, true);
    }
  } catch (...) {
    ctx->stream = main;
    ctx->profiling = prof;
    throw;
  }
  ctx->stream = main;
  ctx->profiling = prof;
  HFG_HIP_CHECK(hipGetLastError());
  HFG_HIP_CHECK(hipEventRecord(ctx->side_ev[1], q));
}

static void eig_sym_batch(hfg_ctx *ctx, EigWork &w, int nblk, const int *ns, const double *const *foldX = nullptr) {
  EigBatch b;
  b.nblk = nblk;
  int nmax = 0;
  for (int i = 0; i < nblk; i++) {
    int n = ns[i];
    nmax = std::max(nmax, n);
    b.n[i] = n;
    w.d[i].resize(n);
    w.e[i].resize(n);
    w.tau[i].resize(n);
    w.v[i].resize(n);
    w.pp[i].resize((size_t)TRD_NCS * n);
    w.dots[i].resize((size_t)TRD_NCS * ((n + 63) / 64) + 8);
    w.Z[i].resize((size_t)n * n);
    long cap = 3L * n * n + 1024;
    w.rot[i].resize(2 * (size_t)cap);
    w.sweeps[i].resize((size_t)4 * 64 * n + 8);
    b.rotcap[i] = cap;
    b.A[i] = w.A[i].p;
    b.d[i] = w.d[i].p;
    b.e[i] = w.e[i].p;
    b.tau[i] = w.tau[i].p;
    b.v[i] = w.v[i].p;
    b.pp[i] = w.pp[i].p;
    b.dots[i] = w.dots[i].p;
    b.Z[i] = w.Z[i].p;
    b.rot[i] = w.rot[i].p;
    b.sweeps[i] = w.sweeps[i].p;
  }
  hipStream_t s = ctx->stream;
  const bool bt_wy = !tuning().bt_column && nmax >= 4 * BT_KB;
  if (tridiagonalize_takes_chain(nblk, ns)) {
    ctx->avoid_side = true;
    ctx->drop_side();
  }
  const bool fold = bt_wy && foldX != nullptr && tuning().bt_fold && !ctx->avoid_side;
  w.folded = fold;
  if (fold)
    for (int i = 0; i < nblk; i++) w.Y[i].resize((size_t)ns[i] * ns[i]);
  if (bt_wy) bt_wy_setup(ctx, w, b, nblk, ns, nmax, fold);
  {
    ProfScope ps(ctx, "eig_tridiag");
    if (tuning().trd_mode == TrdMode::unblocked) {
      size_t shb = (size_t)(nmax + 4 * 64 + 8) * sizeof(double);
      if (shb > 64 * 1024)
        HFG_HIP_CHECK(hipFuncSetAttribute((const void *)k_trd_gemv, hipFuncAttributeMaxDynamicSharedMemorySize, (int)shb));
      for (int k = 0; k <= nmax - 3; k++) {
        int m = nmax - k - 1;
        int nrs = (m + 63) / 64;
        hipLaunchKernelGGL(k_trd_gemv, dim3(nrs * TRD_NCS, nblk), dim3(256), shb, s, b, k);
        hipLaunchKernelGGL(k_trd_update, dim3(nrs * nrs, nblk), dim3(256), 0, s, b, k);
      }
      hipLaunchKernelGGL(k_trd_finish, dim3(nblk), dim3(64), 0, s, b);
    } else {
      double *Ap[MAXB], *dp[MAXB], *ep[MAXB], *tp[MAXB];
      for (int i = 0; i < nblk; i++) {
        Ap[i] = w.A[i].p;
        dp[i] = w.d[i].p;
        ep[i] = w.e[i].p;
        tp[i] = w.tau[i].p;
      }
      tridiagonalize_batch(ctx, nblk, ns, Ap, dp, ep, tp);
    }
  }
  if (bt_wy) bt_wy_prepare(ctx, w, b, nblk, nmax, fold);
  if (fold) bt_wy_fold_x(ctx, w, b, nblk, ns, nmax, foldX);
  {
    ProfScope ps(ctx, "eig_tridiag_solve");
    w.used_dc = !tuning().tridiag_ql;
    if (!w.used_dc) {
      hipLaunchKernelGGL(k_set_identity, dim3((nmax + 255) / 256, nmax, nblk), dim3(256), 0, s, b);
      hipLaunchKernelGGL(k_tql_values, dim3(nblk), dim3(64), 0, s, b);
      hipLaunchKernelGGL(k_tql_apply, dim3((nmax + 63) / 64, nblk), dim3(64), 0, s, b);
    } else {
      double *dp[MAXB], *ep[MAXB], *zp[MAXB];
      for (int i = 0; i < nblk; i++) {
        dp[i] = w.d[i].p;
        ep[i] = w.e[i].p;
        zp[i] = w.Z[i].p;
      }
      tridiag_dc_batch(ctx, nblk, ns, dp, ep, zp);
    }
  }
  {
    ProfScope ps(ctx, "eig_backtransform");
    if (fold) {
      HFG_HIP_CHECK(hipStreamWaitEvent(s, ctx->side_ev[1], 0));
    } else if (bt_wy) {
      bt_wy_apply(ctx, w, b, nblk, nmax);
    } else {
    dim3 grid((nmax + 3) / 4, nblk);
    if (nmax <= 64 * 8)
      hipLaunchKernelGGL(k_backtransform<8>, grid, dim3(256), 0, s, b);
    else if (nmax <= 64 * 24)
      hipLaunchKernelGGL(k_backtransform<24>, grid, dim3(256), 0, s, b);
    else {
      size_t shb = (size_t)4 * nmax * sizeof(double);
      if (shb > 64 * 1024)
        HFG_HIP_CHECK(
            hipFuncSetAttribute((const void *)k_backtransform_lds, hipFuncAttributeMaxDynamicSharedMemorySize, (int)shb));
      hipLaunchKernelGGL(k_backtransform_lds, grid, dim3(256), shb, s, b);
    }
    }
  }
  HFG_HIP_CHECK(hipGetLastError());
}

bool tridiagonalize_takes_chain(int nblk, const int *ns);
void trdp_check_status(hfg_ctx *ctx);
static void check_status(hfg_ctx *ctx, EigWork &w, int nblk) {
  if (w.used_dc) {
    if (dc_status(ctx) != 0) throw std::logic_error("Eigendecomposition failed!\n");
    trdp_check_status(ctx);
    return;
  }
  for (int i = 0; i < nblk; i++) {
    int st[2];
    HFG_HIP_CHECK(hipMemcpyAsync(st, w.sweeps[i].p, 2 * sizeof(int), hipMemcpyDeviceToHost, ctx->stream));
    HFG_HIP_CHECK(hipStreamSynchronize(ctx->stream));
    if (st[1] != 0) throw std::logic_error("Eigendecomposition failed!\n");
  }
}

void eig_sym_dev(hfg_ctx *ctx, int n, const double *dA, double *dE, double *dC) {
  EigWork &w = work_for(ctx);
  w.A[0].resize((size_t)n * n + 2);
  HFG_HIP_CHECK(hipMemcpyAsync(w.A[0].p, dA, sizeof(double) * n * n, hipMemcpyDeviceToDevice, ctx->stream));
  eig_sym_batch(ctx, w, 1, &n);
  DevBuf<int> &rank = w.ibuf1;
  rank.resize(n + 8);
  launch_rank(ctx, w.d[0].p, n, rank.p);
  hipLaunchKernelGGL(k_scatter_cols, dim3((n + 255) / 256, n), dim3(256), 0, ctx->stream, w.Z[0].p, n, n,
                     (const int64_t *)nullptr, rank.p, 0, w.d[0].p, n, dC, dE);
  check_status(ctx, w, 1);
}

void eig_gsym_dev(hfg_ctx *ctx, int N, int n, const double *dF, const double *dS, double *dE, double *dC) {
  EigWork &w = work_for(ctx);
  w.A[0].resize((size_t)n * n + 2);
  DevBuf<double> &T1 = ctx->ws[0];
  DevBuf<double> &Ctmp = ctx->ws[1];
  T1.resize((size_t)N * n);
  Ctmp.resize((size_t)N * n);
  {
    ProfScope ps(ctx, "eig_reduce");
    gemm_dev(ctx, false, false, N, n, N, 1.0, dF, N, dS, N, 0.0, T1.p, N);
    gemm_dev(ctx, true, false, n, n, N, 1.0, dS, N, T1.p, N, 0.0, w.A[0].p, n);
  }
  eig_sym_batch(ctx, w, 1, &n);
  {
    ProfScope ps(ctx, "eig_backtransform");
    gemm_dev(ctx, false, false, N, n, n, 1.0, dS, N, w.Z[0].p, n, 0.0, Ctmp.p, N);
  }
  DevBuf<int> &rank = w.ibuf1;
  rank.resize(n + 8);
  launch_rank(ctx, w.d[0].p, n, rank.p);
  hipLaunchKernelGGL(k_scatter_cols, dim3((N + 255) / 256, n), dim3(256), 0, ctx->stream, Ctmp.p, N, n,
                     (const int64_t *)nullptr, rank.p, 0, w.d[0].p, N, dC, dE);
  check_status(ctx, w, 1);
}

size_t eig_block_buf_size(int nblk, const int64_t *blk_ptr) {
  size_t nmax = 0;
  for (int ib = 0; ib < nblk; ib++) nmax = std::max<size_t>(nmax, blk_ptr[ib + 1] - blk_ptr[ib]);
  return (size_t)nblk * (nmax * nmax + nmax);
}

void eig_blocks_multi_dev(hfg_ctx *ctx, int N, int nF, const double *const *dFs, const double *dS, int nblk, const int64_t *blk_ptr,
                          const int64_t *blk_idx, double *const *dBlockBufs);
static int eig_num_cus(hfg_ctx *ctx) {
  static int ncu = 0;
  if (!ncu) {
    hipDeviceProp_t prop;
    ncu = (hipGetDeviceProperties(&prop, ctx->device) == hipSuccess && prop.multiProcessorCount > 0) ? prop.multiProcessorCount : 256;
  }
  return ncu;
}
void eig_blocks_dev(hfg_ctx *ctx, int N, const double *dF, const double *dS, int nblk, const int64_t *blk_ptr,
                    const int64_t *blk_idx, double *dBlockBuf) {
  eig_blocks_multi_dev(ctx, N, 1, &dF, dS, nblk, blk_ptr, blk_idx, &dBlockBuf);
}
void eig_blocks_multi_dev(hfg_ctx *ctx, int N, int nF, const double *const *dFs, const double *dS, int nblk, const int64_t *blk_ptr,
                          const int64_t *blk_idx, double *const *dBlockBufs) {
  EigWork &w = work_for(ctx);
  hipStream_t s = ctx->stream;
  if (blk_ptr[nblk] != N) throw std::logic_error("Symmetry mismatch in eig_gsym_sub\n");
  DevBuf<double> &idxbuf = w.idx;
  idxbuf.resize(2 * (size_t)N + 16);
  int64_t *drows = (int64_t *)idxbuf.p;
  int64_t *dcols = drows + N;
  for (int ib = 0; ib < nblk; ib++)
    if (blk_ptr[ib + 1] == blk_ptr[ib]) throw std::logic_error("eig_gsym_sub: empty symmetry block\n");
  const bool cached = ctx->fixed_sinvh && ctx->fixed_sinvh == dS && w.sup_S == dS && w.sup_gen == ctx->fixed_gen &&
                      w.sup_N == N &&
                      w.sup_ptr.size() == (size_t)nblk + 1 && std::equal(w.sup_ptr.begin(), w.sup_ptr.end(), blk_ptr) &&
                      w.sup_idx.size() == (size_t)N && std::equal(w.sup_idx.begin(), w.sup_idx.end(), blk_idx);
  if (!cached) {
    w.sup_S = nullptr;
    HFG_HIP_CHECK(hipMemcpyAsync(drows, blk_idx, sizeof(int64_t) * N, hipMemcpyHostToDevice, s));
    DevBuf<int> &flag = w.ibuf2;
    flag.resize((size_t)N * nblk + 8);
    for (int ib = 0; ib < nblk; ib++) {
      int n = (int)(blk_ptr[ib + 1] - blk_ptr[ib]);
      hipLaunchKernelGGL(k_col_support, dim3(N), dim3(256), 0, s, dS, N, drows + blk_ptr[ib], n, flag.p + (size_t)ib * N);
    }
    std::vector<int> hflag((size_t)N * nblk);
    HFG_HIP_CHECK(hipMemcpyAsync(hflag.data(), flag.p, sizeof(int) * hflag.size(), hipMemcpyDeviceToHost, s));
    HFG_HIP_CHECK(hipStreamSynchronize(s));
    std::vector<int64_t> allcols;
    for (int ib = 0; ib < nblk; ib++) {
      int cnt = 0;
      for (int c = 0; c < N; c++)
        if (hflag[(size_t)ib * N + c]) {
          allcols.push_back(c);
          cnt++;
        }
      if (cnt != (int)(blk_ptr[ib + 1] - blk_ptr[ib]))
        throw std::logic_error("eig_gsym_sub: Sinvh is not block structured (columns with support != block size)\n");
    }
    HFG_HIP_CHECK(hipMemcpyAsync(dcols, allcols.data(), sizeof(int64_t) * N, hipMemcpyHostToDevice, s));
    HFG_HIP_CHECK(hipStreamSynchronize(s));
    if (ctx->fixed_sinvh == dS) {
      w.sup_S = dS;
      w.sup_gen = ctx->fixed_gen;
      w.sup_N = N;
      w.sup_ptr.assign(blk_ptr, blk_ptr + nblk + 1);
      w.sup_idx.assign(blk_idx, blk_idx + N);
    }
  }

  size_t nmax = 0;
  for (int ib = 0; ib < nblk; ib++) nmax = std::max<size_t>(nmax, blk_ptr[ib + 1] - blk_ptr[ib]);
  const size_t slot = nmax * nmax + nmax;
  for (int f = 0; f < nF; f++) HFG_HIP_CHECK(hipMemsetAsync(dBlockBufs[f], 0, sizeof(double) * slot * nblk, s));

  std::vector<int> mine;
  for (int f = 0; f < nF; f++)
    for (int ib = 0; ib < nblk; ib++)
      if (ib % ctx->shard_n == ctx->shard_rank) mine.push_back(f * nblk + ib);
  DevBuf<double> &Fb = ctx->ws[5];
  DevBuf<double> &T1 = ctx->ws[0];
  DevBuf<double> &Xall = ctx->ws[4];
  Fb.resize(nmax * nmax * MAXB);
  T1.resize(nmax * nmax * MAXB);
  Xall.resize(nmax * nmax * MAXB);
  for (size_t c0 = 0; c0 < mine.size(); c0 += MAXB) {
    int nb = (int)std::min<size_t>(MAXB, mine.size() - c0);
    std::vector<int> ns(nb);
    std::vector<GemmTask> gt(4 * (size_t)nb);
    const double *Xptr[MAXB];
    int nm = 0;
    for (int k = 0; k < nb; k++) {
      const int ib = mine[c0 + k] % nblk;
      double *dBlockBuf = dBlockBufs[mine[c0 + k] / nblk];
      int n = (int)(blk_ptr[ib + 1] - blk_ptr[ib]);
      ns[k] = n;
      nm = std::max(nm, n);
      w.A[k].resize((size_t)n * n + 2);
      w.Z[k].resize((size_t)n * n);
      w.Y[k].resize((size_t)n * n);
      double *Xb = Xall.p + (size_t)k * nmax * nmax, *Fk = Fb.p + (size_t)k * nmax * nmax, *Tk = T1.p + (size_t)k * nmax * nmax;
      Xptr[k] = Xb;
      GemmTask g;
      g.M = g.N = g.K = n;
      g.lda = g.ldb = g.ldc = n;
      g.A = Fk;
      g.B = Xb;
      g.C = Tk;
      gt[k] = g;
      g.A = Xb;
      g.tA = 1;
      g.B = Tk;
      g.C = w.A[k].p;
      g.sym = 1;
      gt[nb + k] = g;
      g.sym = 0;
      g.tA = 0;
      g.A = Xb;
      g.B = w.Z[k].p;
      g.C = dBlockBuf + (size_t)ib * slot;
      gt[2 * nb + k] = g;
      g.A = w.Y[k].p;
      g.tA = 1;
      gt[3 * nb + k] = g;
    }
    upload_cached(w.gtasks, w.h_gtasks, gt, s);
    {
      ProfScope ps(ctx, "eig_reduce");
      for (int k = 0; k < nb; k++) {
        const int ib = mine[c0 + k] % nblk;
        const double *dF = dFs[mine[c0 + k] / nblk];
        int n = ns[k];
        hipLaunchKernelGGL(k_gather_block, dim3((n + 255) / 256, n), dim3(256), 0, s, dF, dS, N, drows + blk_ptr[ib],
                           dcols + blk_ptr[ib], n, Fb.p + (size_t)k * nmax * nmax, Xall.p + (size_t)k * nmax * nmax);
      }
      const int force_split = tuning().gemm_splitk;
      long full_tiles = 0, low_tiles = 0;
      for (int k = 0; k < nb; k++) {
        const long t1 = (ns[k] + 127) / 128;
        full_tiles += t1 * t1;
        low_tiles += t1 * (t1 + 1) / 2;
      }
      const int slots = 2 * eig_num_cus(ctx);
      const bool split_full = force_split >= 0 ? force_split != 0 : (full_tiles < slots && nm >= 256);
      const bool split_low = force_split >= 0 ? force_split != 0 : (low_tiles < slots && nm >= 256);
      w.split_full = split_full;
      ProfScope pp3(ctx, "eig_products");
      const bool tile64 = force_split < 0 && !gemm_prefers_128(ctx, full_tiles);
      w.tile64 = tile64;
      if (tile64) {
        gemm_tasklist64_dev(ctx, w.gtasks.p, nb, nm, nm);
        gemm_tasklist64_dev(ctx, w.gtasks.p + nb, nb, nm, nm);
        gemm_mirror_lower_dev(ctx, w.gtasks.p + nb, nb, nm);
      } else {
      if (split_full) {
        for (int k = 0; k < nb; k++) HFG_HIP_CHECK(hipMemsetAsync(T1.p + (size_t)k * nmax * nmax, 0, sizeof(double) * (size_t)ns[k] * ns[k], s));
        gemm_tasklist_split2_dev(ctx, w.gtasks.p, nb, nm, nm);
      } else if (tuning().gemm_rect) gemm_tasklist_rect_dev(ctx, w.gtasks.p, nb, nm, nm);
      else gemm_tasklist_dev(ctx, w.gtasks.p, nb, nm, nm);
      if (split_low) {
        for (int k = 0; k < nb; k++) HFG_HIP_CHECK(hipMemsetAsync(w.A[k].p, 0, sizeof(double) * (size_t)ns[k] * ns[k], s));
        gemm_tasklist_split2_dev(ctx, w.gtasks.p + nb, nb, nm, nm);
      } else
        gemm_tasklist_dev(ctx, w.gtasks.p + nb, nb, nm, nm);
      gemm_mirror_lower_dev(ctx, w.gtasks.p + nb, nb, nm);
      }
    }
    eig_sym_batch(ctx, w, nb, ns.data(), Xptr);
    {
      ProfScope ps(ctx, "eig_backtransform");
      {
        ProfScope pp3(ctx, "eig_products");
        const GemmTask *last = w.gtasks.p + (w.folded ? 3 : 2) * (size_t)nb;
        if (w.tile64) gemm_tasklist64_dev(ctx, last, nb, nm, nm);
        else if (w.split_full) gemm_tasklist_split2_dev(ctx, last, nb, nm, nm);
        else if (tuning().gemm_rect) gemm_tasklist_rect_dev(ctx, last, nb, nm, nm);
        else gemm_tasklist_dev(ctx, last, nb, nm, nm);
      }
      std::vector<const double *> csrc;
      std::vector<double *> cdst;
      std::vector<int> cn;
      for (int k = 0; k < nb; k++) {
        const int ib = mine[c0 + k] % nblk;
        double *slotp = dBlockBufs[mine[c0 + k] / nblk] + (size_t)ib * slot;
        csrc.push_back(w.d[k].p);
        cdst.push_back(slotp + nmax * nmax);
        cn.push_back(ns[k]);
      }
      copy_slices(s, csrc, cdst, cn);
    }
    check_status(ctx, w, nb);
  }
  HFG_HIP_CHECK(hipGetLastError());
}

void eig_assemble_dev(hfg_ctx *ctx, int N, int nblk, const int64_t *blk_ptr, const int64_t *blk_idx,
                      const double *dBlockBuf, double *dE, double *dC) {
  EigWork &w = work_for(ctx);
  hipStream_t s = ctx->stream;
  ProfScope ps(ctx, "scatter");
  if (w.asm_rows.size() != (size_t)N || !std::equal(w.asm_rows.begin(), w.asm_rows.end(), blk_idx)) {
    w.asm_rows.assign(blk_idx, blk_idx + N);
    w.asm_rows_dev.resize((size_t)N + 2);
    HFG_HIP_CHECK(hipMemcpyAsync(w.asm_rows_dev.p, w.asm_rows.data(), sizeof(int64_t) * N, hipMemcpyHostToDevice, s));
  }
  int64_t *drows = (int64_t *)w.asm_rows_dev.p;
  size_t nmax = 0;
  for (int ib = 0; ib < nblk; ib++) nmax = std::max<size_t>(nmax, blk_ptr[ib + 1] - blk_ptr[ib]);
  const size_t slot = nmax * nmax + nmax;
  DevBuf<double> &Etmp = ctx->ws[3];
  Etmp.resize(N);
  {
    std::vector<const double *> csrc;
    std::vector<double *> cdst;
    std::vector<int> cn;
    for (int ib = 0; ib < nblk; ib++) {
      csrc.push_back(dBlockBuf + (size_t)ib * slot + nmax * nmax);
      cdst.push_back(Etmp.p + blk_ptr[ib]);
      cn.push_back((int)(blk_ptr[ib + 1] - blk_ptr[ib]));
    }
    copy_slices(s, csrc, cdst, cn);
  }
  DevBuf<int> &rank = w.ibuf1;
  rank.resize(N + 8);
  HFG_HIP_CHECK(hipMemsetAsync(dC, 0, sizeof(double) * (size_t)N * N, s));
  launch_rank(ctx, Etmp.p, N, rank.p);
  for (int ib = 0; ib < nblk; ib++) {
    int n = (int)(blk_ptr[ib + 1] - blk_ptr[ib]);
    hipLaunchKernelGGL(k_scatter_cols, dim3((n + 255) / 256, n), dim3(256), 0, s, dBlockBuf + (size_t)ib * slot, n, n,
                       drows + blk_ptr[ib], rank.p, (int)blk_ptr[ib], Etmp.p + blk_ptr[ib], N, dC, dE);
  }
  HFG_HIP_CHECK(hipGetLastError());
}

void eig_gsym_sub_dev(hfg_ctx *ctx, int N, const double *dF, const double *dS, int nblk, const int64_t *blk_ptr,
                      const int64_t *blk_idx, double *dE, double *dC) {
  int save_rank = ctx->shard_rank, save_n = ctx->shard_n;
  ctx->shard_rank = 0;
  ctx->shard_n = 1;
  try {
    DevBuf<double> &buf = ctx->ws[6];
    buf.resize(eig_block_buf_size(nblk, blk_ptr));
    eig_blocks_dev(ctx, N, dF, dS, nblk, blk_ptr, blk_idx, buf.p);
    eig_assemble_dev(ctx, N, nblk, blk_ptr, blk_idx, buf.p, dE, dC);
  } catch (...) {
    ctx->shard_rank = save_rank;
    ctx->shard_n = save_n;
    throw;
  }
  ctx->shard_rank = save_rank;
  ctx->shard_n = save_n;
}

void eig_block_supports(hfg_ctx *ctx, int N, const double *dS, int nblk, const int64_t *blk_ptr, const int64_t *blk_idx,
                        std::vector<int64_t> &cols) {
  hipStream_t s = ctx->stream;
  DevBuf<int64_t> drows;
  DevBuf<int> flag;
  drows.resize(N);
  flag.resize((size_t)N * nblk + 8);
  HFG_HIP_CHECK(hipMemcpyAsync(drows.p, blk_idx, sizeof(int64_t) * N, hipMemcpyHostToDevice, s));
  for (int ib = 0; ib < nblk; ib++) {
    const int n = (int)(blk_ptr[ib + 1] - blk_ptr[ib]);
    hipLaunchKernelGGL(k_col_support, dim3(N), dim3(256), 0, s, dS, N, drows.p + blk_ptr[ib], n, flag.p + (size_t)ib * N);
  }
  std::vector<int> hflag((size_t)N * nblk);
  HFG_HIP_CHECK(hipMemcpyAsync(hflag.data(), flag.p, sizeof(int) * hflag.size(), hipMemcpyDeviceToHost, s));
  HFG_HIP_CHECK(hipStreamSynchronize(s));
  cols.clear();
  for (int ib = 0; ib < nblk; ib++) {
    int cnt = 0;
    for (int c = 0; c < N; c++)
      if (hflag[(size_t)ib * N + c]) {
        cols.push_back(c);
        cnt++;
      }
    if (cnt != (int)(blk_ptr[ib + 1] - blk_ptr[ib]))
      throw std::logic_error("eig_gsym_sub: Sinvh is not block structured (columns with support != block size)\n");
  }
}

void eig_gsym_sub_pair_dev(hfg_ctx *ctx, int N, const double *dFa, const double *dFb, const double *dS, int nblk, const int64_t *blk_ptr,
                           const int64_t *blk_idx, double *dEa, double *dCa, double *dEb, double *dCb) {
  int save_rank = ctx->shard_rank, save_n = ctx->shard_n;
  ctx->shard_rank = 0;
  ctx->shard_n = 1;
  try {
    const size_t sz = eig_block_buf_size(nblk, blk_ptr);
    DevBuf<double> &buf = ctx->ws[6];
    buf.resize(2 * sz);
    const double *Fs[2] = {dFa, dFb};
    double *bufs[2] = {buf.p, buf.p + sz};
    eig_blocks_multi_dev(ctx, N, 2, Fs, dS, nblk, blk_ptr, blk_idx, bufs);
    eig_assemble_dev(ctx, N, nblk, blk_ptr, blk_idx, bufs[0], dEa, dCa);
    eig_assemble_dev(ctx, N, nblk, blk_ptr, blk_idx, bufs[1], dEb, dCb);
  } catch (...) {
    ctx->shard_rank = save_rank;
    ctx->shard_n = save_n;
    throw;
  }
  ctx->shard_rank = save_rank;
  ctx->shard_n = save_n;
}

}
```

helfem_amd/csrc/hip/gemm.hip:

```cpp
#include "common.h"
#include <algorithm>
#include <cstdint>
#include <cstdlib>
#include <cstring>

namespace hfg {

typedef double double4_t __attribute__((ext_vector_type(4)));
typedef double d2_t __attribute__((ext_vector_type(2)));

template <int BM, int BN, bool ACC = false, int MF = 1>
__device__ __forceinline__ void dgemm_tile(int id, int transA, int transB, int M, int N, int K, double alpha,
                                           const double *__restrict__ A, int lda, const double *__restrict__ B, int ldb,
                                           double beta, double *__restrict__ C, int ldc, double (*As)[16][BM + 16],
                                           double (*Bs)[16][BN + 16], int sym = 0, int kbeg = 0, int kend = -1, int over = 0) {
  constexpr int BK = 16;
  constexpr int PAD = 16;
  constexpr int WM = BM / 2, WN = BN / 2;
  constexpr int TM = WM / 16, TN = WN / 16;
  static_assert(PAD == 16, "LDS row padding is part of the tile types");

  int nbm = (M + BM - 1) / BM, nbn = (N + BN - 1) / BN;
  const bool lower = !ACC && sym == 1;
  int nwg = lower ? nbm * (nbm + 1) / 2 : nbm * nbn;
  if (!(over & 4)) {
    int q = nwg / 8, r = nwg % 8, xcd = id % 8;
    id = (xcd < r ? xcd * (q + 1) : r * (q + 1) + (xcd - r) * q) + id / 8;
  }
  int bm = (id % nbm) * BM, bn = (id / nbm) * BN;
  if (lower) {
    int ti = (int)((sqrt(8.0 * (double)id + 1.0) - 1.0) * 0.5);
    while (ti * (ti + 1) / 2 > id) ti--;
    while ((ti + 1) * (ti + 2) / 2 <= id) ti++;
    const int tj = id - ti * (ti + 1) / 2;
    if (ti >= nbm) return;
    bm = ti * BM;
    bn = tj * BN;
  }

  if constexpr (ACC) {
    if (sym == 2 && bm / BM + 3 < bn / BN) return;
  }
  const int tid = threadIdx.x, wave = tid >> 6, lane = tid & 63;
  const int wm = (wave & 1) * WM, wn = (wave >> 1) * WN;
  const int l15 = lane & 15, l4 = lane >> 4;

  constexpr bool V4 = (MF == 1);
  double4_t accv[V4 ? TM : 1][V4 ? TN : 1];
  double accs[V4 ? 1 : TM][V4 ? 1 : TN][4];
  if constexpr (V4) {
#pragma unroll
    for (int i = 0; i < TM; i++)
#pragma unroll
      for (int j = 0; j < TN; j++) accv[i][j] = (double4_t){0.0, 0.0, 0.0, 0.0};
  } else {
#pragma unroll
    for (int i = 0; i < TM; i++)
#pragma unroll
      for (int j = 0; j < TN; j++)
#pragma unroll
        for (int c = 0; c < 4; c++) accs[i][j][c] = 0.0;
  }
  auto acc = [&](int i, int j, int r) -> double {
    if constexpr (V4) return accv[i][j][r];
    else return accs[i][j][r];
  };

  constexpr bool PRE = ACC && (TM * TN <= 4);
  double cpre[PRE ? TM : 1][PRE ? TN : 1][4];
  if constexpr (PRE) {
#pragma unroll
    for (int i = 0; i < TM; i++)
#pragma unroll
      for (int j = 0; j < TN; j++)
#pragma unroll
        for (int r = 0; r < 4; r++) {
          int gm = min(bm + wm + i * 16 + l15, M - 1), gn = min(bn + wn + j * 16 + l4 + 4 * r, N - 1);
          cpre[i][j][r] = C[(size_t)gn * ldc + gm];
        }
  }

  constexpr int VA = BM * BK / 2 / 256, VB = BN * BK / 2 / 256;
  const bool fastA = ((reinterpret_cast<uintptr_t>(A) & 15) == 0) && ((lda & 1) == 0) && (bm + BM <= M || (over & 1));
  const bool fastB = ((reinterpret_cast<uintptr_t>(B) & 15) == 0) && ((ldb & 1) == 0) && (bn + BN <= N || (over & 2));
  const int a_mv = tid % (BM / 2), a_kc = tid / (BM / 2);
  const int a_m = tid % BM, a_kv = tid / BM;
  const int b_nv = tid % (BN / 2), b_kc = tid / (BN / 2);
  const int b_n = tid % BN, b_kv = tid / BN;
  const double *pA = transA ? A + (size_t)(bm + a_m) * lda + 2 * a_kv : A + (size_t)a_kc * lda + bm + 2 * a_mv;
  const double *pB = transB ? B + (size_t)b_kc * ldb + bn + 2 * b_nv : B + (size_t)(bn + b_n) * ldb + 2 * b_kv;
  d2_t va[VA], vb[VB];
  auto load_tiles = [&](int k0) {
    const bool fullk = (k0 + BK <= K);
    if (fastA && fullk) {
      if (!transA) {
#pragma unroll
        for (int r = 0; r < VA; r++) va[r] = *reinterpret_cast<const d2_t *>(pA + (size_t)(k0 + r * (512 / BM)) * lda);
      } else {
#pragma unroll
        for (int r = 0; r < VA; r++) va[r] = *reinterpret_cast<const d2_t *>(pA + k0 + 2 * r * (256 / BM));
      }
    } else {
#pragma unroll
      for (int r = 0; r < VA; r++) {
        int gm0, gk0, gm1, gk1;
        if (!transA) {
          gm0 = bm + 2 * a_mv;
          gm1 = gm0 + 1;
          gk0 = gk1 = k0 + a_kc + r * (512 / BM);
        } else {
          gm0 = gm1 = bm + a_m;
          gk0 = k0 + 2 * (a_kv + r * (256 / BM));
          gk1 = gk0 + 1;
        }
        d2_t v;
        v.x = (gm0 < M && gk0 < K) ? (transA ? A[(size_t)gm0 * lda + gk0] : A[(size_t)gk0 * lda + gm0]) : 0.0;
        v.y = (gm1 < M && gk1 < K) ? (transA ? A[(size_t)gm1 * lda + gk1] : A[(size_t)gk1 * lda + gm1]) : 0.0;
        va[r] = v;
      }
    }
    if (fastB && fullk) {
      if (transB) {
#pragma unroll
        for (int r = 0; r < VB; r++) vb[r] = *reinterpret_cast<const d2_t *>(pB + (size_t)(k0 + r * (512 / BN)) * ldb);
      } else {
#pragma unroll
        for (int r = 0; r < VB; r++) vb[r] = *reinterpret_cast<const d2_t *>(pB + k0 + 2 * r * (256 / BN));
      }
    } else {
#pragma unroll
      for (int r = 0; r < VB; r++) {
        int gn0, gk0, gn1, gk1;
        if (transB) {
          gn0 = bn + 2 * b_nv;
          gn1 = gn0 + 1;
          gk0 = gk1 = k0 + b_kc + r * (512 / BN);
        } else {
          gn0 = gn1 = bn + b_n;
          gk0 = k0 + 2 * (b_kv + r * (256 / BN));
          gk1 = gk0 + 1;
        }
        d2_t v;
        v.x = (gn0 < N && gk0 < K) ? (transB ? B[(size_t)gk0 * ldb + gn0] : B[(size_t)gn0 * ldb + gk0]) : 0.0;
        v.y = (gn1 < N && gk1 < K) ? (transB ? B[(size_t)gk1 * ldb + gn1] : B[(size_t)gn1 * ldb + gk1]) : 0.0;
        vb[r] = v;
      }
    }
  };
  auto store_tiles = [&](int buf) {
    if (!transA) {
#pragma unroll
      for (int r = 0; r < VA; r++) *reinterpret_cast<d2_t *>(&As[buf][a_kc + r * (512 / BM)][2 * a_mv]) = va[r];
    } else {
#pragma unroll
      for (int r = 0; r < VA; r++) {
        As[buf][2 * (a_kv + r * (256 / BM))][a_m] = va[r].x;
        As[buf][2 * (a_kv + r * (256 / BM)) + 1][a_m] = va[r].y;
      }
    }
    if (transB) {
#pragma unroll
      for (int r = 0; r < VB; r++) *reinterpret_cast<d2_t *>(&Bs[buf][b_kc + r * (512 / BN)][2 * b_nv]) = vb[r];
    } else {
#pragma unroll
      for (int r = 0; r < VB; r++) {
        Bs[buf][2 * (b_kv + r * (256 / BN))][b_n] = vb[r].x;
        Bs[buf][2 * (b_kv + r * (256 / BN)) + 1][b_n] = vb[r].y;
      }
    }
  };

  const bool splitk = kend >= 0;
  const int kstop = splitk ? min(kend, K) : K;
  load_tiles(kbeg);
  store_tiles(0);
  __syncthreads();
  int buf = 0;
  for (int k0 = kbeg; k0 < kstop; k0 += BK) {
    const bool more = (k0 + BK < kstop);
    if (more) load_tiles(k0 + BK);
#pragma unroll
    for (int kk = 0; kk < BK; kk += 4) {
      double fa[TM];
#pragma unroll
      for (int i = 0; i < TM; i++) fa[i] = As[buf][kk + l4][wm + i * 16 + l15];
      if constexpr (MF == 1) {
        double fb[TN];
#pragma unroll
        for (int j = 0; j < TN; j++) fb[j] = Bs[buf][kk + l4][wn + j * 16 + l15];
#pragma unroll
        for (int i = 0; i < TM; i++)
#pragma unroll
          for (int j = 0; j < TN; j++)
            accv[i][j] = __builtin_amdgcn_mfma_f64_16x16x4f64(fb[j], fa[i], accv[i][j], 0, 0, 0);
      } else {
#pragma unroll
        for (int j = 0; j < TN; j++) {
          double fb[4];
#pragma unroll
          for (int c = 0; c < 4; c++) fb[c] = Bs[buf][kk + l4][wn + j * 16 + 4 * c + (lane & 3)];
#pragma unroll
          for (int i = 0; i < TM; i++)
#pragma unroll
            for (int c = 0; c < 4; c++)
              accs[i][j][c] = __builtin_amdgcn_mfma_f64_4x4x4f64(fb[c], fa[i], accs[i][j][c], 0, 0, 0);
        }
      }
    }
    if (more) store_tiles(buf ^ 1);
    __syncthreads();
    buf ^= 1;
  }
  if constexpr (PRE) {
#pragma unroll
    for (int i = 0; i < TM; i++)
#pragma unroll
      for (int j = 0; j < TN; j++)
#pragma unroll
        for (int r = 0; r < 4; r++) {
          int gm = bm + wm + i * 16 + l15, gn = bn + wn + j * 16 + l4 + 4 * r;
          if (gm < M && gn < N) C[(size_t)gn * ldc + gm] = alpha * acc(i, j, r) + beta * cpre[i][j][r];
        }
    return;
  } else if constexpr (ACC) {
    constexpr int HI = (TM > 2) ? TM / 2 : TM;
#pragma unroll
    for (int i0 = 0; i0 < TM; i0 += HI) {
      double cv[HI][TN][4];
#pragma unroll
      for (int i = 0; i < HI; i++)
#pragma unroll
        for (int j = 0; j < TN; j++)
#pragma unroll
          for (int r = 0; r < 4; r++) {
            int gm = min(bm + wm + (i0 + i) * 16 + l15, M - 1), gn = min(bn + wn + j * 16 + l4 + 4 * r, N - 1);
            cv[i][j][r] = C[(size_t)gn * ldc + gm];
          }
#pragma unroll
      for (int i = 0; i < HI; i++)
#pragma unroll
        for (int j = 0; j < TN; j++)
#pragma unroll
          for (int r = 0; r < 4; r++) {
            int gm = bm + wm + (i0 + i) * 16 + l15, gn = bn + wn + j * 16 + l4 + 4 * r;
            if (gm < M && gn < N) C[(size_t)gn * ldc + gm] = alpha * acc(i0 + i, j, r) + beta * cv[i][j][r];
          }
    }
    return;
  }
#pragma unroll
  for (int i = 0; i < TM; i++)
#pragma unroll
    for (int j = 0; j < TN; j++)
#pragma unroll
      for (int r = 0; r < 4; r++) {
        int gm = bm + wm + i * 16 + l15, gn = bn + wn + j * 16 + l4 + 4 * r;
        if (gm < M && gn < N) {
          size_t o = (size_t)gn * ldc + gm;
          double v = alpha * acc(i, j, r);
          if (splitk) {
            unsafeAtomicAdd(&C[o], v);
            continue;
          }
          if (beta != 0.0) v += beta * C[o];
          C[o] = v;
        }
      }
}

template <int BM, int BN, int MF = 1>
__global__ __launch_bounds__(256, 2) void k_dgemm(int transA, int transB, int M, int N, int K, double alpha,
                                               const double *__restrict__ A, int lda, const double *__restrict__ B,
                                               int ldb, double beta, double *__restrict__ C, int ldc) {
  __shared__ __attribute__((aligned(16))) double As[2][16][BM + 16];
  __shared__ __attribute__((aligned(16))) double Bs[2][16][BN + 16];
  dgemm_tile<BM, BN, false, MF>(blockIdx.x, transA, transB, M, N, K, alpha, A, lda, B, ldb, beta, C, ldc, As, Bs);
}

template <int BM, int BN, bool ACC = false, int MF = 1>
__global__ __launch_bounds__(256, 2) void k_dgemm_tasklist(const GemmTask *__restrict__ tasks) {
  __shared__ __attribute__((aligned(16))) double As[2][16][BM + 16];
  __shared__ __attribute__((aligned(16))) double Bs[2][16][BN + 16];
  const GemmTask t = tasks[blockIdx.y];
  if (t.M <= 0 || t.N <= 0) return;
  const int sym = (!ACC && BM == BN && t.M == t.N && t.beta == 0.0) ? (t.sym == 1) : ((ACC && t.sym == 2) ? 2 : 0);
  const int nbm = (t.M + BM - 1) / BM;
  const int nt = (sym == 1) ? nbm * (nbm + 1) / 2 : nbm * ((t.N + BN - 1) / BN);
  if ((int)blockIdx.x >= nt) return;
  dgemm_tile<BM, BN, ACC, MF>(blockIdx.x, t.tA, t.tB, t.M, t.N, t.K, t.alpha, t.A, t.lda, t.B, t.ldb, t.beta, t.C, t.ldc,
                              As, Bs, sym, 0, -1, t.over);
}

template <int BM, int BN, bool SPLIT = false>
__global__ __launch_bounds__(256, 2) void k_dgemm_tasklist_wl(const GemmTask *__restrict__ tasks, const int2 *__restrict__ wl, int nwg) {
  __shared__ __attribute__((aligned(16))) double As[2][16][BM + 16];
  __shared__ __attribute__((aligned(16))) double Bs[2][16][BN + 16];
  const int xcd = blockIdx.x % 8, slot = blockIdx.x / 8;
  const int q8 = nwg / 8, r8 = nwg % 8;
  if (slot >= q8 + (xcd < r8 ? 1 : 0)) return;
  const int2 w = wl[(xcd < r8 ? xcd * (q8 + 1) : r8 * (q8 + 1) + (xcd - r8) * q8) + slot];
  const GemmTask t = tasks[w.x];
  if constexpr (SPLIT) {
    const int half = w.y & 1;
    const int Kh = ((t.K / 2 + 15) / 16) * 16;
    const int kbeg = half ? Kh : 0, kend = half ? t.K : Kh;
    if (kbeg >= kend) return;
    dgemm_tile<BM, BN, false, 1>(w.y >> 1, t.tA, t.tB, t.M, t.N, t.K, t.alpha, t.A, t.lda, t.B, t.ldb, 0.0, t.C, t.ldc, As, Bs, 0, kbeg,
                                 kend, t.over | 4);
  } else {
    dgemm_tile<BM, BN, false, 1>(w.y, t.tA, t.tB, t.M, t.N, t.K, t.alpha, t.A, t.lda, t.B, t.ldb, t.beta, t.C, t.ldc, As, Bs, 0, 0, -1,
                                 t.over | 4);
  }
}

template <int BM, int BN>
__global__ __launch_bounds__(256, 2) void k_dgemm_tasklist_split2(const GemmTask *__restrict__ tasks) {
  __shared__ __attribute__((aligned(16))) double As[2][16][BM + 16];
  __shared__ __attribute__((aligned(16))) double Bs[2][16][BN + 16];
  const GemmTask t = tasks[blockIdx.y];
  if (t.M <= 0 || t.N <= 0) return;
  const int sym = (BM == BN && t.M == t.N) ? (t.sym == 1) : 0;
  const int nbm = (t.M + BM - 1) / BM;
  const int nt = (sym == 1) ? nbm * (nbm + 1) / 2 : nbm * ((t.N + BN - 1) / BN);
  const int tile = blockIdx.x >> 1, half = blockIdx.x & 1;
  if (tile >= nt) return;
  const int Kh = ((t.K / 2 + 15) / 16) * 16;
  const int kbeg = half ? Kh : 0, kend = half ? t.K : Kh;
  if (kbeg >= kend) return;
  dgemm_tile<BM, BN, false, 1>(tile, t.tA, t.tB, t.M, t.N, t.K, t.alpha, t.A, t.lda, t.B, t.ldb, 0.0, t.C, t.ldc, As, Bs, sym, kbeg, kend);
}

static bool mfma4() { return tuning().mfma_4x4x4; }

void gemm_tasklist_acc_dev(hfg_ctx *ctx, const GemmTask *dtasks, int ntasks, int maxM, int maxN, bool tile64) {
  if (ntasks <= 0 || maxM <= 0 || maxN <= 0) return;
  ProfScope ps(ctx, "gemm");
  if (tile64) {
    const int tiles = ((maxM + 63) / 64) * ((maxN + 63) / 64);
    if (mfma4()) hipLaunchKernelGGL((k_dgemm_tasklist<64, 64, true, 0>), dim3(tiles, ntasks), dim3(256), 0, ctx->stream, dtasks);
    else hipLaunchKernelGGL((k_dgemm_tasklist<64, 64, true>), dim3(tiles, ntasks), dim3(256), 0, ctx->stream, dtasks);
  } else {
    const int tiles = ((maxM + 127) / 128) * ((maxN + 127) / 128);
    if (mfma4()) hipLaunchKernelGGL((k_dgemm_tasklist<128, 128, true, 0>), dim3(tiles, ntasks), dim3(256), 0, ctx->stream, dtasks);
    else hipLaunchKernelGGL((k_dgemm_tasklist<128, 128, true>), dim3(tiles, ntasks), dim3(256), 0, ctx->stream, dtasks);
  }
  HFG_HIP_CHECK(hipGetLastError());
}

__global__ __launch_bounds__(256) void k_mirror_lower(const GemmTask *__restrict__ tasks) {
  __shared__ double tile[64][65];
  const GemmTask t = tasks[blockIdx.y];
  if (t.sym != 1 || t.M <= 0 || t.M != t.N) return;
  const int nb = (t.M + 63) / 64;
  int bi = (int)((1.0 + sqrt(1.0 + 8.0 * (double)blockIdx.x)) * 0.5);
  while (bi * (bi - 1) / 2 > (int)blockIdx.x) bi--;
  while ((bi + 1) * bi / 2 <= (int)blockIdx.x) bi++;
  const int bj = blockIdx.x - bi * (bi - 1) / 2;
  if (bi >= nb) return;
  const int tx = threadIdx.x & 63, ty = threadIdx.x >> 6;
  for (int c = ty; c < 64; c += 4) {
    int gm = bi * 64 + tx, gn = bj * 64 + c;
    tile[c][tx] = (gm < t.M && gn < t.N) ? t.C[(size_t)gn * t.ldc + gm] : 0.0;
  }
  __syncthreads();
  for (int c = ty; c < 64; c += 4) {
    int gm = bj * 64 + tx, gn = bi * 64 + c;
    if (gm < t.M && gn < t.N) t.C[(size_t)gn * t.ldc + gm] = tile[tx][c];
  }
}

void gemm_mirror_lower_dev(hfg_ctx *ctx, const GemmTask *dtasks, int ntasks, int maxN) {
  if (ntasks <= 0 || maxN <= 64) return;
  const int nb = (maxN + 63) / 64;
  hipLaunchKernelGGL(k_mirror_lower, dim3(nb * (nb - 1) / 2, ntasks), dim3(256), 0, ctx->stream, dtasks);
  HFG_HIP_CHECK(hipGetLastError());
}

void gemm_tasklist64_dev(hfg_ctx *ctx, const GemmTask *dtasks, int ntasks, int maxM, int maxN) {
  if (ntasks <= 0 || maxM <= 0 || maxN <= 0) return;
  ProfScope ps(ctx, "gemm");
  const int tiles = ((maxM + 63) / 64) * ((maxN + 63) / 64);
  if (mfma4()) hipLaunchKernelGGL((k_dgemm_tasklist<64, 64, false, 0>), dim3(tiles, ntasks), dim3(256), 0, ctx->stream, dtasks);
  else hipLaunchKernelGGL((k_dgemm_tasklist<64, 64>), dim3(tiles, ntasks), dim3(256), 0, ctx->stream, dtasks);
  HFG_HIP_CHECK(hipGetLastError());
}

void gemm_tasklist_rect_dev(hfg_ctx *ctx, const GemmTask *dtasks, int ntasks, int maxM, int maxN) {
  if (ntasks <= 0 || maxM <= 0 || maxN <= 0) return;
  ProfScope ps(ctx, "gemm");
  const int tiles = ((maxM + 127) / 128) * ((maxN + 63) / 64);
  hipLaunchKernelGGL((k_dgemm_tasklist<128, 64>), dim3(tiles, ntasks), dim3(256), 0, ctx->stream, dtasks);
  HFG_HIP_CHECK(hipGetLastError());
}

void gemm_tasklist_split2_dev(hfg_ctx *ctx, const GemmTask *dtasks, int ntasks, int maxM, int maxN) {
  if (ntasks <= 0 || maxM <= 0 || maxN <= 0) return;
  ProfScope ps(ctx, "gemm");
  const int tiles = ((maxM + 127) / 128) * ((maxN + 127) / 128);
  hipLaunchKernelGGL((k_dgemm_tasklist_split2<128, 128>), dim3(2 * tiles, ntasks), dim3(256), 0, ctx->stream, dtasks);
  HFG_HIP_CHECK(hipGetLastError());
}

void gemm_tasklist_wl_dev(hfg_ctx *ctx, const GemmTask *dtasks, const int2 *dwl, int nwg, int tiles) {
  if (nwg <= 0) return;
  ProfScope ps(ctx, "gemm");
  const unsigned grid = 8u * (unsigned)((nwg + 7) / 8);
  if (tiles == 2) hipLaunchKernelGGL((k_dgemm_tasklist_wl<64, 64>), dim3(grid), dim3(256), 0, ctx->stream, dtasks, dwl, nwg);
  else if (tiles == 1) hipLaunchKernelGGL((k_dgemm_tasklist_wl<128, 64>), dim3(grid), dim3(256), 0, ctx->stream, dtasks, dwl, nwg);
  else hipLaunchKernelGGL((k_dgemm_tasklist_wl<128, 128>), dim3(grid), dim3(256), 0, ctx->stream, dtasks, dwl, nwg);
  HFG_HIP_CHECK(hipGetLastError());
}

void gemm_tasklist_wl_split2_rect_dev(hfg_ctx *ctx, const GemmTask *dtasks, const int2 *dwl, int nwg) {
  if (nwg <= 0) return;
  ProfScope ps(ctx, "gemm");
  hipLaunchKernelGGL((k_dgemm_tasklist_wl<128, 64, true>), dim3(8u * (unsigned)((nwg + 7) / 8)), dim3(256), 0, ctx->stream, dtasks, dwl, nwg);
  HFG_HIP_CHECK(hipGetLastError());
}

void gemm_tasklist_split2_rect_dev(hfg_ctx *ctx, const GemmTask *dtasks, int ntasks, int maxM, int maxN) {
  if (ntasks <= 0 || maxM <= 0 || maxN <= 0) return;
  ProfScope ps(ctx, "gemm");
  const int tiles = ((maxM + 127) / 128) * ((maxN + 63) / 64);
  hipLaunchKernelGGL((k_dgemm_tasklist_split2<128, 64>), dim3(2 * tiles, ntasks), dim3(256), 0, ctx->stream, dtasks);
  HFG_HIP_CHECK(hipGetLastError());
}

bool gemm_prefers_128(hfg_ctx *ctx, long tiles128);
void gemm_tasklist_dev(hfg_ctx *ctx, const GemmTask *dtasks, int ntasks, int maxM, int maxN) {
  if (ntasks <= 0 || maxM <= 0 || maxN <= 0) return;
  const int tiles = ((maxM + 127) / 128) * ((maxN + 127) / 128);
  if (ntasks <= 65535 && !gemm_prefers_128(ctx, (long)ntasks * tiles)) {
    gemm_tasklist64_dev(ctx, dtasks, ntasks, maxM, maxN);
    return;
  }
  ProfScope ps(ctx, "gemm");
  for (int t0 = 0; t0 < ntasks; t0 += 65535) {
    int nt = std::min(65535, ntasks - t0);
    if (mfma4()) hipLaunchKernelGGL((k_dgemm_tasklist<128, 128, false, 0>), dim3(tiles, nt), dim3(256), 0, ctx->stream, dtasks + t0);
    else hipLaunchKernelGGL((k_dgemm_tasklist<128, 128>), dim3(tiles, nt), dim3(256), 0, ctx->stream, dtasks + t0);
  }
  HFG_HIP_CHECK(hipGetLastError());
}

bool gemm_prefers_128(hfg_ctx *ctx, long tiles128) {
  if (tuning().gemm_tile) return tuning().gemm_tile == 128;
  static int slots = 0;
  if (!slots) {
    int ncu = 256;
    (void)hipDeviceGetAttribute(&ncu, hipDeviceAttributeMultiprocessorCount, ctx->device);
    slots = 2 * ncu;
  }
  const long rounds = (tiles128 + slots - 1) / slots;
  return tiles128 >= slots / 2 && (double)tiles128 >= 0.85 * (double)(rounds * slots);
}

void gemm_dev(hfg_ctx *ctx, bool tA, bool tB, int M, int N, int K, double alpha, const double *A, int lda,
              const double *B, int ldb, double beta, double *C, int ldc) {
  if (M <= 0 || N <= 0) return;
  ProfScope ps(ctx, "gemm");
  long big_tiles = (long)((M + 127) / 128) * ((N + 127) / 128);
  if (gemm_prefers_128(ctx, big_tiles)) {
    if (mfma4())
      hipLaunchKernelGGL((k_dgemm<128, 128, 0>), dim3((unsigned)big_tiles), dim3(256), 0, ctx->stream, (int)tA, (int)tB, M, N, K,
                         alpha, A, lda, B, ldb, beta, C, ldc);
    else
      hipLaunchKernelGGL((k_dgemm<128, 128>), dim3((unsigned)big_tiles), dim3(256), 0, ctx->stream, (int)tA, (int)tB, M, N, K,
                         alpha, A, lda, B, ldb, beta, C, ldc);
  } else {
    long tiles = (long)((M + 63) / 64) * ((N + 63) / 64);
    if (mfma4())
      hipLaunchKernelGGL((k_dgemm<64, 64, 0>), dim3((unsigned)tiles), dim3(256), 0, ctx->stream, (int)tA, (int)tB, M, N, K, alpha, A,
                         lda, B, ldb, beta, C, ldc);
    else
      hipLaunchKernelGGL((k_dgemm<64, 64>), dim3((unsigned)tiles), dim3(256), 0, ctx->stream, (int)tA, (int)tB, M, N, K, alpha, A,
                         lda, B, ldb, beta, C, ldc);
  }
  HFG_HIP_CHECK(hipGetLastError());
}

}
```

helfem_amd/csrc/host/tuning.h:

```cpp
#pragma once
#include <string>

namespace helfem {
constexpr int EXL_GMAX = 16;
enum class TrdMode { persistent, chain, twokernel, unblocked };
#define HELFEM_TUNING(X) \
  X(scf_host, bool, false, "HELFEM_SCF", true, "=host", !strcmp(e, "host"), "SCF loop driven from the host through the per-stage entry points (checker of the device-resident loop)") \
  X(tei_host, bool, false, "HELFEM_TEI", false, "=host", !strcmp(e, "host"), "in-element tables built by the threaded host code and uploaded (checker of tei_dev.hip)") \
  X(exchange_general, bool, false, "HELFEM_EXCHANGE", true, "=general", !strcmp(e, "general"), "general exchange kernels always, not only where the low-rank fast path declines") \
  X(exl_rb, int, 0, "HELFEM_EXL_RB", false, "int", atoi(e), "RB kernel of the low-rank exchange: 4 the 4 x 4 vector kernel, 1 the one-pair vector kernel (checkers), else the matrix-core kernel k_exl_RBm") \
  X(exl_mgroups, bool, true, "HELFEM_EXL_MGROUPS", false, "off if 0", atoi(e) != 0, "cross-element products by blocks of equal m; off: the full products") \
  X(exl_rect, int, -1, "HELFEM_EXL_RECT", false, "int", atoi(e), "tiles of the element GEMM: 0 / 1 / 2 = 128 x 128 / 128 x 64 / 64 x 64 always; negative: 64 x 64 when the tasks average fewer than 1500 pairs, else 128 x 128") \
  X(exl_wl, bool, true, "HELFEM_EXL_WL", false, "off if 0", atoi(e) != 0, "XCD-contiguous workgroup lists for the element GEMM and the cross products; off: plain task-list grids") \
  X(exl_splitk, bool, true, "HELFEM_EXL_SPLITK", false, "off if 0", atoi(e) != 0, "two half-K workgroups per tile for the cross products; off: one workgroup per tile") \
  X(exl_crect, bool, true, "HELFEM_EXL_CRECT", false, "off if 0", atoi(e) != 0, "128 x 64 tiles for the split cross products; off: 128 x 128") \
  X(exl_groups, int, 4, "HELFEM_EXL_GROUPS", false, "int", std::max(1, std::min(EXL_GMAX, atoi(e))), "groups of 64 factors tried before the general kernels take over, clamped to 1 ... 16") \
  X(exl_hint, bool, true, "HELFEM_EXL_HINT", false, "off if 0", atoi(e) != 0, "the SCF loop's occupied orbitals taken as the factors of P; off: always factorise and verify P (checker)") \
  X(exl_pair, bool, true, "HELFEM_EXL_PAIR", false, "off if 0", atoi(e) != 0, "low-rank fast path for the pair (erfc) tables; off: general kernels") \
  X(fock_overlap, bool, true, "HELFEM_FOCK_OVERLAP", false, "off if 0", atoi(e) != 0, "Coulomb kernels on the side stream beside the XC kernels; off: one after the other on the main stream") \
  X(xc_lds_limit, size_t, 150 * 1024, "HELFEM_XC_LDS_LIMIT", false, "int", (size_t)atol(e), "bytes of LDS the angular XC kernels plan with; smaller forces the chunked kernels (tests)") \
  X(diis_blocks, bool, true, "HELFEM_DIIS_BLOCKS", false, "off if 0", atoi(e) != 0, "DIIS error per symmetry block; off: the four dense N^3 products (checker)") \
  X(diis_lowrank, bool, true, "HELFEM_DIIS_LOWRANK", false, "off if 0", atoi(e) != 0, "blocked DIIS error from the occupied orbitals; off: per-block n^3 products from F and P (checker)") \
  X(eig_pair, bool, true, "HELFEM_EIG_PAIR", false, "off if 0", atoi(e) != 0, "both spins' Fock matrices in one batched eigensolve; off: two calls") \
  X(trd_mode, TrdMode, TrdMode::persistent, "HELFEM_TRD", false, "word", !strcmp(e, "persistent") ? TrdMode::persistent : !strcmp(e, "twokernel") ? TrdMode::twokernel : !strcmp(e, "unblocked") ? TrdMode::unblocked : TrdMode::chain, "tridiagonalisation: persistent = k_trdp where the batch fits, else the chain; chain (and any unknown word) = one k_trdf launch per column always (checker); twokernel = k_trdb_gemv + k_trdb_w; unblocked = the first-generation kernels") \
  X(trdp_min, int, 256, "HELFEM_TRDP_MIN", false, "int", atoi(e), "smallest order the persistent kernel takes") \
  X(trdp_r, int, 0, "HELFEM_TRDP_R", false, "int", atoi(e), "rows per thread of the persistent kernel forced (0: the first that fits)") \
  X(trdp_u, int, 0, "HELFEM_TRDP_U", false, "int", atoi(e), "column chunks per thread of the persistent kernel forced wider than needed (measurement; 0: narrowest)") \
  X(trdp_limit_ms, long long, 200, "HELFEM_TRDP_LIMIT_MS", false, "int", atoll(e), "wall-clock bound of every spin of the persistent kernel, ms") \
  X(trdp_phases, bool, true, "HELFEM_TRDP_PHASES", false, "off if 0", atoi(e) != 0, "one cooperative launch per phase; off: the whole matrix in one launch (checker)") \
  X(trdp_step, int, 96, "HELFEM_TRDP_STEP", false, "int", std::max(1, atoi(e)), "fewest columns of a phase (at least 1)") \
  X(trdp_coop, bool, true, "HELFEM_TRDP_COOP", false, "off if 0", atoi(e) != 0, "hipLaunchCooperativeKernel for the phases; off: plain launches (A/B of the launch overhead)") \
  X(trdp_stamps, int, 0, "HELFEM_TRDP_STAMPS", false, "int", atoi(e), "non-zero: the stamping kernels, one launch per eigensolve, phase summary on stderr; 2 and more: also per-column stamps of one workgroup") \
  X(trdp_stamps_file, std::string, "", "HELFEM_TRDP_STAMPS_FILE", false, "path", e, "with stamps: file for the stamps of every workgroup over 64 columns (tools/trdp_window.py)") \
  X(trd_tail, int, 2, "HELFEM_TRD_TAIL", false, "int", atoi(e), "last columns of the chain in one launch: 0 none, 1 the LDS-resident kernel (order 128), else the register-resident kernel (order 192)") \
  X(trdf_sym, int, -1, "HELFEM_TRDF_SYM", false, "int", atoi(e), "symmetric sweep of k_trdf: 0 never, other non-negative always, negative by HELFEM_TRDF_SYM_MIN") \
  X(trdf_sym_min, int, 0, "HELFEM_TRDF_SYM_MIN", false, "int", atoi(e), "panels whose full grid has more tiles than this sweep one triangle only") \
  X(trd_band_update, bool, true, "HELFEM_TRD_BAND_UPDATE", false, "off if 0", atoi(e) != 0, "band-limited trailing updates when every sweep is symmetric; off: full updates") \
  X(trdf_nth, int, 0, "HELFEM_TRDF_NTH", false, "int", atoi(e), "512: k_trdf with 512 threads; anything else 1024 (A/B runs)") \
  X(acc_tile, int, 0, "HELFEM_ACC_TILE", false, "int", atoi(e), "128: 128 x 128 tiles for the accumulating updates (and full, not band-limited ones); anything else 64 x 64") \
  X(trdf_dbg, int, 0, "HELFEM_TRDF_DBG", false, "int", atoi(e), "measurement replay of k_trdf only: bits 0-2 go to the kernel's debug field, bit 2 also prints the per-wave stamps (tools/trdf_probe.py)") \
  X(trdf_c, int, -1, "HELFEM_TRDF_C", false, "int", atoi(e), "measurement replay of k_trdf only: column-in-panel index forced for every launch (negative: each launch's own)") \
  X(tridiag_ql, bool, false, "HELFEM_TRIDIAG", false, "=ql", !strcmp(e, "ql"), "one-lane implicit QL for the tridiagonal problem instead of divide and conquer (checker)") \
  X(dc_gemm_small, bool, false, "HELFEM_DC_GEMM", false, "=small", !strcmp(e, "small"), "Q U of the divide-and-conquer merges by the first 64 x 64 kernel instead of the tile engine (checker)") \
  X(dc_dbg, bool, false, "HELFEM_DC_DBG", false, "present", true, "merge statistics of divide and conquer on stderr") \
  X(bt_column, bool, false, "HELFEM_BT", false, "=column", !strcmp(e, "column"), "back-transformation reflector by reflector instead of compact WY (checker)") \
  X(bt_fold, bool, true, "HELFEM_BT_FOLD", false, "off if 0", atoi(e) != 0, "X Q formed on the side stream beside divide and conquer; off: Z <- Q Z on the main stream behind it") \
  X(bt_side, bool, false, "HELFEM_BT_SIDE", false, "=1", atoi(e) == 1, "without the fold: the compact-WY set-up on the side stream") \
  X(gemm_tile, int, 0, "HELFEM_GEMM_TILE", false, "int", atoi(e), "128: 128 x 128 tiles always; other non-zero: 64 x 64 always; 0: the large tiles where they fill whole rounds of the chip") \
  X(gemm_splitk, int, -1, "HELFEM_GEMM_SPLITK", false, "int", atoi(e), "eigensolve's products: 0 / other non-negative = large tiles without / with two half-K workgroups each; negative: chosen by tile count") \
  X(gemm_rect, bool, false, "HELFEM_GEMM_RECT", false, "on if not 0", atoi(e) != 0, "128 x 64 tiles for the eigensolve's large-tile products") \
  X(mfma_4x4x4, bool, false, "HELFEM_MFMA", false, "=4x4x4", !strcmp(e, "4x4x4"), "v_mfma_f64_4x4x4_4b_f64 in the tile engine instead of v_mfma_f64_16x16x4_f64 (A/B runs)") \
  X(num_threads, int, 0, "HELFEM_NUM_THREADS", true, "int", std::max(0, atoi(e)), "host threads of the set-up code (0: one per core, 64 at most)") \
  X(hdf5_lib, std::string, "", "HELFEM_HDF5_LIB", true, "path", e, "HDF5 library tried before the usual names")

struct Tuning {
#define X(field, type, def, ...) type field = def;
  HELFEM_TUNING(X)
#undef X
};
const Tuning &tuning();
Tuning tuning_live();
std::string tuning_table();
}
```

Before: 8.682 ms.

## Ping-pong divide-and-conquer Q buffers with column-mapped GEMM instead of gather/scatter

The divide-and-conquer merge no longer gathers the non-deflated columns of Q into a compact buffer, multiplies, and scatters or copies them back. Instead Q alternates between two buffers by tree depth. The product reads and writes columns through index maps (amap and cmap) inside the GEMM tile loaders, and deflated columns are placed directly by a new kernel fused with U construction. zhat and rank are also fused into one launch, and the initial memset of Z is dropped, which cuts several passes over Q and several launches per level. The eigenproduct launch is moved after copy_slices. The indirect column loads may reduce coalescing, and the old path remains available as a checker option.

```diff
diff --git a/helfem_amd/csrc/hip/common.h b/helfem_amd/csrc/hip/common.h
--- a/helfem_amd/csrc/hip/common.h
+++ b/helfem_amd/csrc/hip/common.h
@@ -131,8 +131,9 @@
   double alpha = 1.0, beta = 0.0;
   int sym = 0;
   int over = 0;
+  const int *amap = nullptr, *cmap = nullptr;
 };
-static_assert(sizeof(GemmTask) == 80, "GemmTask is compared bytewise: keep it free of padding");
+static_assert(sizeof(GemmTask) == 96, "GemmTask is compared bytewise: keep it free of padding");
 
 struct ProfScope {
   hfg_ctx *c;
diff --git a/helfem_amd/csrc/hip/dc.hip b/helfem_amd/csrc/hip/dc.hip
--- a/helfem_amd/csrc/hip/dc.hip
+++ b/helfem_amd/csrc/hip/dc.hip
@@ -10,6 +10,9 @@
 
 struct DCNode {
   int blk, lo, mid, hi;
+  int par;
+  int plo, phi;
+  int pad;
 };
 
 struct DCBatch {
@@ -23,7 +26,13 @@
   double *rotc[DC_MAXB], *rots[DC_MAXB];
   int *src[DC_MAXB], *flag[DC_MAXB], *nd[DC_MAXB], *org[DC_MAXB], *roti[DC_MAXB], *rotj[DC_MAXB], *rank[DC_MAXB];
   int *ndpos[DC_MAXB];
+  int *acol[DC_MAXB], *ccol[DC_MAXB];
 };
+
+__device__ __forceinline__ int dc_win(const DCNode &nd, int pp) { return pp ? (nd.par ^ 1) : 0; }
+__device__ __forceinline__ int dc_wout(const DCNode &nd, int pp) { return pp ? nd.par : 1; }
+__device__ __forceinline__ double *dc_Q(const DCBatch &b, int blk, int w) { return w ? b.Qb[blk] : b.Qa[blk]; }
+__device__ __forceinline__ double *dc_d(const DCBatch &b, int blk, int w) { return w ? b.d2[blk] : b.d[blk]; }
 
 __global__ void k_dc_tear(DCBatch b, const DCNode *__restrict__ nodes, int nnodes, double *__restrict__ rho) {
   int i = blockIdx.x * blockDim.x + threadIdx.x;
@@ -36,7 +45,7 @@
 }
 
 __global__ __launch_bounds__(64) void k_dc_leaf(DCBatch b, const DCNode *__restrict__ leaves, int nleaves,
-                                                int *__restrict__ status) {
+                                                int *__restrict__ status, int pp) {
   __shared__ double ds[DC_LEAF], es[DC_LEAF], zt[DC_LEAF][DC_LEAF + 1];
   int li = blockIdx.x;
   if (li >= nleaves) return;
@@ -110,9 +119,14 @@
     double v = ds[lane];
     int rk = 0;
     for (int j = 0; j < s; j++) rk += (ds[j] < v) || (ds[j] == v && j < lane);
-    d[lo + rk] = v;
-    double *Q = b.Qa[lf.blk];
-    for (int k = 0; k < s; k++) Q[(size_t)(lo + rk) * ld + lo + k] = zt[lane][k];
+    const int wl = pp ? lf.par : 0;
+    dc_d(b, lf.blk, wl)[lo + rk] = v;
+    double *Q = dc_Q(b, lf.blk, wl) + (size_t)(lo + rk) * ld;
+    for (int k = 0; k < s; k++) Q[lo + k] = zt[lane][k];
+    if (pp) {
+      for (int r = lf.plo; r < lo; r++) Q[r] = 0.0;
+      for (int r = lf.hi; r < lf.phi; r++) Q[r] = 0.0;
+    }
   }
 }
 
@@ -121,7 +135,7 @@
                                                     const double *__restrict__ rho_all, int node0,
                                                     int *__restrict__ kcount, int *__restrict__ nrot,
                                                     double *__restrict__ rho_eff, GemmTask *__restrict__ tasks,
-                                                    double *__restrict__ gscratch, size_t gstride) {
+                                                    double *__restrict__ gscratch, size_t gstride, int pp) {
   extern __shared__ double lds_[];
   double *sh = gscratch ? gscratch + (size_t)blockIdx.x * gstride : lds_;
   const int ni = node0 + blockIdx.x;
@@ -140,8 +154,8 @@
   __shared__ double red[8];
   __shared__ double tol_sh;
   __shared__ int k_sh;
-  const double *d = b.d[blk];
-  const double *Q = b.Qa[blk];
+  const double *d = dc_d(b, blk, dc_win(nd, pp));
+  const double *Q = dc_Q(b, blk, dc_win(nd, pp));
   const double rs = rho_all[ni];
   const double sgn = (rs >= 0.0) ? 1.0 : -1.0;
   const double rho = 2.0 * fabs(rs);
@@ -331,9 +345,16 @@
     nrot[ni] = nr;
     rho_eff[ni] = rho;
     GemmTask t;
-    t.A = b.Qg[blk] + (size_t)lo * ld + lo;
+    if (pp) {
+      t.A = Q + lo;
+      t.C = dc_Q(b, blk, dc_wout(nd, pp)) + lo;
+      t.amap = b.acol[blk] + lo;
+      t.cmap = b.ccol[blk] + lo;
+    } else {
+      t.A = b.Qg[blk] + (size_t)lo * ld + lo;
+      t.C = b.Qn[blk] + (size_t)lo * ld + lo;
+    }
     t.B = b.U[blk] + (size_t)lo * ld + lo;
-    t.C = b.Qn[blk] + (size_t)lo * ld + lo;
     t.M = n;
     t.N = k;
     t.K = k;
@@ -380,13 +401,14 @@
     int sidx = snd[c];
     b.ndpos[blk][lo + sidx] = c;
     b.nd[blk][lo + c] = sidx;
+    b.acol[blk][lo + c] = lo + ssrc[sidx];
     b.dnd[blk][lo + c] = sD[sidx];
     b.znd[blk][lo + c] = sz[sidx];
   }
 }
 
 __global__ __launch_bounds__(256) void k_dc_rotate(DCBatch b, const DCNode *__restrict__ nodes, int node0,
-                                                   const int *__restrict__ nrot) {
+                                                   const int *__restrict__ nrot, int pp) {
   const int ni = node0 + blockIdx.y;
   const DCNode nd = nodes[ni];
   const int nr = nrot[ni];
@@ -397,7 +419,7 @@
   __shared__ int scp[256], scj[256];
   __shared__ double sc[256], ss[256];
   const int *src = b.src[blk] + lo;
-  double *Q = b.Qa[blk] + lo + r;
+  double *Q = dc_Q(b, blk, dc_win(nd, pp)) + lo + r;
   for (int t0 = 0; t0 < nr; t0 += 256) {
     const int t = t0 + threadIdx.x;
     if (t < nr) {
@@ -514,11 +536,10 @@
   }
 }
 
-__global__ __launch_bounds__(256) void k_dc_zhat(DCBatch b, const DCNode *__restrict__ nodes, int node0,
-                                                 const int *__restrict__ kcount, const double *__restrict__ rho_eff) {
-  const int ni = node0 + blockIdx.y;
+__device__ __forceinline__ void dc_zhat_body(const DCBatch &b, const DCNode *__restrict__ nodes, int ni, int bx,
+                                             const int *__restrict__ kcount, const double *__restrict__ rho_eff) {
   const int k = kcount[ni];
-  const int j = blockIdx.x * 4 + (threadIdx.x >> 6);
+  const int j = bx * 4 + (threadIdx.x >> 6);
   if (j >= k) return;
   const int lane = threadIdx.x & 63;
   const DCNode nd = nodes[ni];
@@ -537,12 +558,15 @@
     b.zhat[blk][lo + j] = (b.znd[blk][lo + j] >= 0.0) ? zh : -zh;
   }
 }
-
-__global__ __launch_bounds__(256) void k_dc_U(DCBatch b, const DCNode *__restrict__ nodes, int node0,
-                                              const int *__restrict__ kcount) {
-  const int ni = node0 + blockIdx.y;
+__global__ __launch_bounds__(256) void k_dc_zhat(DCBatch b, const DCNode *__restrict__ nodes, int node0,
+                                                 const int *__restrict__ kcount, const double *__restrict__ rho_eff) {
+  dc_zhat_body(b, nodes, node0 + blockIdx.y, blockIdx.x, kcount, rho_eff);
+}
+
+__device__ __forceinline__ void dc_U_body(const DCBatch &b, const DCNode *__restrict__ nodes, int ni, int bx,
+                                          const int *__restrict__ kcount) {
   const int k = kcount[ni];
-  const int i = blockIdx.x * 4 + (threadIdx.x >> 6);
+  const int i = bx * 4 + (threadIdx.x >> 6);
   if (i >= k) return;
   const int lane = threadIdx.x & 63;
   const DCNode nd = nodes[ni];
@@ -558,6 +582,37 @@
   s = 1.0 / sqrt(wave_sum(s));
   double *Ucol = b.U[blk] + (size_t)(lo + i) * ld + lo;
   for (int j = lane; j < k; j += 64) Ucol[j] = zh[j] / ((d[j] - dorg) - mui) * s;
+}
+__global__ __launch_bounds__(256) void k_dc_U(DCBatch b, const DCNode *__restrict__ nodes, int node0,
+                                              const int *__restrict__ kcount) {
+  dc_U_body(b, nodes, node0 + blockIdx.y, blockIdx.x, kcount);
+}
+
+constexpr int DC_PSL = 8;
+__global__ __launch_bounds__(256) void k_dc_U_place(DCBatch b, const DCNode *__restrict__ nodes, int node0,
+                                                    const int *__restrict__ kcount, int nU, int nPx) {
+  const int ni = node0 + blockIdx.y;
+  if ((int)blockIdx.x < nU) {
+    dc_U_body(b, nodes, ni, blockIdx.x, kcount);
+    return;
+  }
+  const DCNode nd = nodes[ni];
+  const int q = blockIdx.x - nU, s0 = (q / nPx) * DC_PSL;
+  const int blk = nd.blk, lo = nd.lo, hi = nd.hi;
+  if (s0 >= hi - lo) return;
+  const int r = nd.plo + (q % nPx) * 256 + threadIdx.x;
+  if (r >= nd.phi) return;
+  const int ld = b.n[blk];
+  const bool inside = r >= lo && r < hi;
+  double *qout = dc_Q(b, blk, dc_wout(nd, 1));
+  const double *qin = dc_Q(b, blk, dc_win(nd, 1));
+  const int s1 = min(s0 + DC_PSL, hi - lo);
+  for (int s = s0; s < s1; s++) {
+    const bool defl = b.flag[blk][lo + s] != 0;
+    if (inside && !defl) continue;
+    const double v = inside ? qin[(size_t)(lo + b.src[blk][lo + s]) * ld + r] : 0.0;
+    qout[(size_t)(lo + b.rank[blk][lo + s]) * ld + r] = v;
+  }
 }
 
 __global__ void k_dc_gather(DCBatch b, const DCNode *__restrict__ nodes, int node0,
@@ -577,19 +632,17 @@
   b.Qg[blk][(size_t)(lo + c) * ld + lo + r] = Q[(size_t)col * ld + lo + r];
 }
 
-__global__ __launch_bounds__(256) void k_dc_rank(DCBatch b, const DCNode *__restrict__ nodes, int node0,
-                                                 const int *__restrict__ kcount) {
-  extern __shared__ double sh[];
-  const int ni = node0 + blockIdx.x;
+__device__ __forceinline__ void dc_rank_body(const DCBatch &b, const DCNode *__restrict__ nodes, int ni, int slice,
+                                             double *__restrict__ sh, int pp) {
   const DCNode nd = nodes[ni];
   const int blk = nd.blk, lo = nd.lo, n = nd.hi - nd.lo;
-  if ((int)blockIdx.y * 32 >= n) return;
+  if (slice * 32 >= n) return;
   const int *flag = b.flag[blk] + lo;
   for (int s = threadIdx.x; s < n; s += blockDim.x) {
     sh[s] = flag[s] ? b.Ds[blk][lo + s] : b.lam[blk][lo + b.ndpos[blk][lo + s]];
   }
   __syncthreads();
-  const int s = blockIdx.y * 32 + (threadIdx.x >> 3), part = threadIdx.x & 7;
+  const int s = slice * 32 + (threadIdx.x >> 3), part = threadIdx.x & 7;
   const int per = (n + 7) >> 3, j0 = part * per, j1 = min(n, j0 + per);
   const bool ok = s < n;
   const double v = ok ? sh[s] : 0.0;
@@ -613,8 +666,22 @@
   rk += __builtin_amdgcn_update_dpp(0, rk, 0x141, 0xf, 0xf, true);
   if (ok && part == 0) {
     b.rank[blk][lo + s] = rk;
-    b.d2[blk][lo + rk] = v;
-  }
+    dc_d(b, blk, dc_wout(nd, pp))[lo + rk] = v;
+    if (pp && !flag[s]) b.ccol[blk][lo + b.ndpos[blk][lo + s]] = lo + rk;
+  }
+}
+__global__ __launch_bounds__(256) void k_dc_rank(DCBatch b, const DCNode *__restrict__ nodes, int node0,
+                                                 const int *__restrict__ kcount) {
+  extern __shared__ double sh[];
+  dc_rank_body(b, nodes, node0 + blockIdx.x, blockIdx.y, sh, 0);
+}
+__global__ __launch_bounds__(256) void k_dc_zhat_rank(DCBatch b, const DCNode *__restrict__ nodes, int node0,
+                                                      const int *__restrict__ kcount, const double *__restrict__ rho_eff,
+                                                      int nZ) {
+  extern __shared__ double sh[];
+  const int ni = node0 + blockIdx.y;
+  if ((int)blockIdx.x < nZ) dc_zhat_body(b, nodes, ni, blockIdx.x, kcount, rho_eff);
+  else dc_rank_body(b, nodes, ni, blockIdx.x - nZ, sh, 1);
 }
 
 __global__ void k_dc_scatter(DCBatch b, const DCNode *__restrict__ nodes, int node0, const int *__restrict__ kcount) {
@@ -659,6 +726,7 @@
 }
 
 void gemm_tasklist64_dev(hfg_ctx *ctx, const GemmTask *dtasks, int ntasks, int maxM, int maxN);
+void gemm_tasklist64_map_dev(hfg_ctx *ctx, const GemmTask *dtasks, int ntasks, int maxM, int maxN);
 typedef double double4_t __attribute__((ext_vector_type(4)));
 
 __global__ __launch_bounds__(256) void k_dgemm_tasks(const GemmTask *__restrict__ tasks) {
@@ -684,7 +752,7 @@
       int e = tid + 256 * r;
       int m = e % BM, kk = e / BM;
       int gm = bm + m, gk = k0 + kk;
-      As[kk][m] = (gm < M && gk < K) ? t.A[(size_t)gk * t.lda + gm] : 0.0;
+      As[kk][m] = (gm < M && gk < K) ? t.A[(size_t)(t.amap ? t.amap[gk] : gk) * t.lda + gm] : 0.0;
       int k2 = e % BK, n2 = e / BK;
       int gn = bn + n2, gk2 = k0 + k2;
       Bs[k2][n2] = (gn < N && gk2 < K) ? t.B[(size_t)gn * t.ldb + gk2] : 0.0;
@@ -703,7 +771,7 @@
     for (int j = 0; j < 2; j++)
       for (int r = 0; r < 4; r++) {
         int gm = bm + wm + i * 16 + l15, gn = bn + wn + j * 16 + l4 + 4 * r;
-        if (gm < M && gn < N) t.C[(size_t)gn * t.ldc + gm] = acc[i][j][r];
+        if (gm < M && gn < N) t.C[(size_t)(t.cmap ? t.cmap[gn] : gn) * t.ldc + gm] = acc[i][j][r];
       }
 }
 
@@ -729,6 +797,7 @@
   std::vector<DCNode> hnodes;
   std::vector<int> level_off;
   std::vector<int> level_maxn;
+  std::vector<int> level_maxp;
   int nleaves = 0;
 };
 static std::map<hfg_ctx *, DCWork *> g_dc;
@@ -740,11 +809,15 @@
   }
 }
 
-static int build_tree(int blk, int lo, int hi, std::vector<std::vector<DCNode> > &byheight) {
+static int build_tree(int blk, int lo, int hi, int depth, int plo, int phi, std::vector<std::vector<DCNode> > &byheight) {
   DCNode nd;
   nd.blk = blk;
   nd.lo = lo;
   nd.hi = hi;
+  nd.par = depth & 1;
+  nd.plo = plo;
+  nd.phi = phi;
+  nd.pad = 0;
   if (hi - lo <= DC_LEAF) {
     nd.mid = lo;
     if (byheight.empty()) byheight.resize(1);
@@ -753,7 +826,7 @@
   }
   int mid = lo + (hi - lo) / 2;
   nd.mid = mid;
-  int h = 1 + std::max(build_tree(blk, lo, mid, byheight), build_tree(blk, mid, hi, byheight));
+  int h = 1 + std::max(build_tree(blk, lo, mid, depth + 1, lo, hi, byheight), build_tree(blk, mid, hi, depth + 1, lo, hi, byheight));
   if ((int)byheight.size() <= h) byheight.resize(h + 1);
   byheight[h].push_back(nd);
   return h;
@@ -773,17 +846,22 @@
   std::vector<int> key(ns, ns + nblk);
   if (key != w.key) {
     std::vector<std::vector<DCNode> > byh;
-    for (int b = 0; b < nblk; b++) build_tree(b, 0, ns[b], byh);
+    for (int b = 0; b < nblk; b++) build_tree(b, 0, ns[b], 0, 0, ns[b], byh);
     w.hnodes.clear();
     w.level_off.clear();
     w.level_maxn.clear();
+    w.level_maxp.clear();
     w.hnodes.insert(w.hnodes.end(), byh[0].begin(), byh[0].end());
     w.nleaves = (int)byh[0].size();
     for (size_t h = 1; h < byh.size(); h++) {
       w.level_off.push_back((int)w.hnodes.size());
-      int mx = 0;
-      for (auto &nd : byh[h]) mx = std::max(mx, nd.hi - nd.lo);
+      int mx = 0, mp = 0;
+      for (auto &nd : byh[h]) {
+        mx = std::max(mx, nd.hi - nd.lo);
+        mp = std::max(mp, nd.phi - nd.plo);
+      }
       w.level_maxn.push_back(mx);
+      w.level_maxp.push_back(mp);
       w.hnodes.insert(w.hnodes.end(), byh[h].begin(), byh[h].end());
     }
     w.level_off.push_back((int)w.hnodes.size());
@@ -800,6 +878,7 @@
   }
   DCBatch b;
   int nmax = 0;
+  const int pp = tuning().dc_levels ? 0 : 1;
   for (int i = 0; i < nblk; i++) {
     int n = ns[i];
     nmax = std::max(nmax, n);
@@ -807,10 +886,12 @@
     w.d2[i].resize(n);
     w.Qb[i].resize(nn);
     w.U[i].resize(nn);
-    w.Qg[i].resize(nn);
-    w.Qn[i].resize(nn);
+    if (!pp) {
+      w.Qg[i].resize(nn);
+      w.Qn[i].resize(nn);
+    }
     w.vec[i].resize((size_t)9 * n);
-    w.ivec[i].resize((size_t)8 * n);
+    w.ivec[i].resize((size_t)10 * n);
     b.n[i] = n;
     b.d[i] = d[i];
     b.d2[i] = w.d2[i].p;
@@ -839,14 +920,16 @@
     b.rotj[i] = iv + 5 * n;
     b.rank[i] = iv + 6 * n;
     b.ndpos[i] = iv + 7 * n;
-    HFG_HIP_CHECK(hipMemsetAsync(Z[i], 0, sizeof(double) * nn, s));
+    b.acol[i] = iv + 8 * n;
+    b.ccol[i] = iv + 9 * n;
+    if (!pp) HFG_HIP_CHECK(hipMemsetAsync(Z[i], 0, sizeof(double) * nn, s));
   }
   HFG_HIP_CHECK(hipMemsetAsync(w.status.p, 0, sizeof(int) * 4, s));
   const int ninternal = (int)w.hnodes.size() - w.nleaves;
   if (ninternal > 0)
     hipLaunchKernelGGL(k_dc_tear, dim3((ninternal + 255) / 256), dim3(256), 0, s, b, w.nodes.p + w.nleaves, ninternal,
                        w.rho.p + w.nleaves);
-  hipLaunchKernelGGL(k_dc_leaf, dim3(w.nleaves), dim3(64), 0, s, b, w.nodes.p, w.nleaves, w.status.p);
+  hipLaunchKernelGGL(k_dc_leaf, dim3(w.nleaves), dim3(64), 0, s, b, w.nodes.p, w.nleaves, w.status.p, pp);
   const int nlevels = (int)w.level_off.size() - 1;
   for (int h = 0; h < nlevels; h++) {
     const int node0 = w.level_off[h], nn = w.level_off[h + 1] - node0;
@@ -862,10 +945,25 @@
     } else if (shb > 64 * 1024)
       HFG_HIP_CHECK(hipFuncSetAttribute((const void *)k_dc_prepare, hipFuncAttributeMaxDynamicSharedMemorySize, (int)shb));
     hipLaunchKernelGGL(k_dc_prepare, dim3(nn), dim3(256), shb, s, b, w.nodes.p, w.rho.p, node0, w.kcount.p, w.nrot.p,
-                       w.rho_eff.p, w.tasks.p, gscr, gstride);
-    hipLaunchKernelGGL(k_dc_rotate, dim3((mx + 255) / 256, nn), dim3(256), 0, s, b, w.nodes.p, node0, w.nrot.p);
+                       w.rho_eff.p, w.tasks.p, gscr, gstride, pp);
+    hipLaunchKernelGGL(k_dc_rotate, dim3((mx + 255) / 256, nn), dim3(256), 0, s, b, w.nodes.p, node0, w.nrot.p, pp);
     hipLaunchKernelGGL(k_dc_secular, dim3((mx + 3) / 4, nn), dim3(256), 0, s, b, w.nodes.p, node0, w.kcount.p,
                        w.rho_eff.p);
+    size_t shr = (size_t)mx * sizeof(double);
+    if (pp) {
+      const int nZ = (mx + 3) / 4, nPx = (w.level_maxp[h] + 255) / 256;
+      if (shr > 64 * 1024)
+        HFG_HIP_CHECK(hipFuncSetAttribute((const void *)k_dc_zhat_rank, hipFuncAttributeMaxDynamicSharedMemorySize, (int)shr));
+      hipLaunchKernelGGL(k_dc_zhat_rank, dim3(nZ + (mx + 31) / 32, nn), dim3(256), shr, s, b, w.nodes.p, node0, w.kcount.p,
+                         w.rho_eff.p, nZ);
+      hipLaunchKernelGGL(k_dc_U_place, dim3(nZ + nPx * ((mx + DC_PSL - 1) / DC_PSL), nn), dim3(256), 0, s, b, w.nodes.p, node0, w.kcount.p, nZ,
+                         nPx);
+      if (tuning().dc_gemm_small)
+        hipLaunchKernelGGL(k_dgemm_tasks, dim3(((mx + 63) / 64) * ((mx + 63) / 64), nn), dim3(256), 0, s, w.tasks.p);
+      else
+        gemm_tasklist64_map_dev(ctx, w.tasks.p, nn, mx, mx);
+      continue;
+    }
     hipLaunchKernelGGL(k_dc_zhat, dim3((mx + 3) / 4, nn), dim3(256), 0, s, b, w.nodes.p, node0, w.kcount.p, w.rho_eff.p);
     hipLaunchKernelGGL(k_dc_U, dim3((mx + 3) / 4, nn), dim3(256), 0, s, b, w.nodes.p, node0, w.kcount.p);
     hipLaunchKernelGGL(k_dc_gather, dim3((mx + 255) / 256, mx, nn), dim3(256), 0, s, b, w.nodes.p, node0, w.kcount.p);
@@ -874,7 +972,6 @@
       hipLaunchKernelGGL(k_dgemm_tasks, dim3(tiles, nn), dim3(256), 0, s, w.tasks.p);
     } else
       gemm_tasklist64_dev(ctx, w.tasks.p, nn, mx, mx);
-    size_t shr = (size_t)mx * sizeof(double);
     if (shr > 64 * 1024)
       HFG_HIP_CHECK(hipFuncSetAttribute((const void *)k_dc_rank, hipFuncAttributeMaxDynamicSharedMemorySize, (int)shr));
     hipLaunchKernelGGL(k_dc_rank, dim3(nn, (mx + 31) / 32), dim3(256), shr, s, b, w.nodes.p, node0, w.kcount.p);
diff --git a/helfem_amd/csrc/hip/eig.hip b/helfem_amd/csrc/hip/eig.hip
--- a/helfem_amd/csrc/hip/eig.hip
+++ b/helfem_amd/csrc/hip/eig.hip
@@ -1226,14 +1226,6 @@
     eig_sym_batch(ctx, w, nb, ns.data(), Xptr);
     {
       ProfScope ps(ctx, "eig_backtransform");
-      {
-        ProfScope pp3(ctx, "eig_products");
-        const GemmTask *last = w.gtasks.p + (w.folded ? 3 : 2) * (size_t)nb;
-        if (w.tile64) gemm_tasklist64_dev(ctx, last, nb, nm, nm);
-        else if (w.split_full) gemm_tasklist_split2_dev(ctx, last, nb, nm, nm);
-        else if (tuning().gemm_rect) gemm_tasklist_rect_dev(ctx, last, nb, nm, nm);
-        else gemm_tasklist_dev(ctx, last, nb, nm, nm);
-      }
       std::vector<const double *> csrc;
       std::vector<double *> cdst;
       std::vector<int> cn;
@@ -1245,6 +1237,14 @@
         cn.push_back(ns[k]);
       }
       copy_slices(s, csrc, cdst, cn);
+      {
+        ProfScope pp3(ctx, "eig_products");
+        const GemmTask *last = w.gtasks.p + (w.folded ? 3 : 2) * (size_t)nb;
+        if (w.tile64) gemm_tasklist64_dev(ctx, last, nb, nm, nm);
+        else if (w.split_full) gemm_tasklist_split2_dev(ctx, last, nb, nm, nm);
+        else if (tuning().gemm_rect) gemm_tasklist_rect_dev(ctx, last, nb, nm, nm);
+        else gemm_tasklist_dev(ctx, last, nb, nm, nm);
+      }
     }
     check_status(ctx, w, nb);
   }
diff --git a/helfem_amd/csrc/hip/gemm.hip b/helfem_amd/csrc/hip/gemm.hip
--- a/helfem_amd/csrc/hip/gemm.hip
+++ b/helfem_amd/csrc/hip/gemm.hip
@@ -9,11 +9,12 @@
 typedef double double4_t __attribute__((ext_vector_type(4)));
 typedef double d2_t __attribute__((ext_vector_type(2)));
 
-template <int BM, int BN, bool ACC = false, int MF = 1>
+template <int BM, int BN, bool ACC = false, int MF = 1, bool MAP = false>
 __device__ __forceinline__ void dgemm_tile(int id, int transA, int transB, int M, int N, int K, double alpha,
                                            const double *__restrict__ A, int lda, const double *__restrict__ B, int ldb,
                                            double beta, double *__restrict__ C, int ldc, double (*As)[16][BM + 16],
-                                           double (*Bs)[16][BN + 16], int sym = 0, int kbeg = 0, int kend = -1, int over = 0) {
+                                           double (*Bs)[16][BN + 16], int sym = 0, int kbeg = 0, int kend = -1, int over = 0,
+                                           const int *__restrict__ amap = nullptr, const int *__restrict__ cmap = nullptr) {
   constexpr int BK = 16;
   constexpr int PAD = 16;
   constexpr int WM = BM / 2, WN = BN / 2;
@@ -87,12 +88,29 @@
   const int a_m = tid % BM, a_kv = tid / BM;
   const int b_nv = tid % (BN / 2), b_kc = tid / (BN / 2);
   const int b_n = tid % BN, b_kv = tid / BN;
-  const double *pA = transA ? A + (size_t)(bm + a_m) * lda + 2 * a_kv : A + (size_t)a_kc * lda + bm + 2 * a_mv;
+  const double *pA = MAP ? A + bm + 2 * a_mv : transA ? A + (size_t)(bm + a_m) * lda + 2 * a_kv : A + (size_t)a_kc * lda + bm + 2 * a_mv;
   const double *pB = transB ? B + (size_t)b_kc * ldb + bn + 2 * b_nv : B + (size_t)(bn + b_n) * ldb + 2 * b_kv;
   d2_t va[VA], vb[VB];
   auto load_tiles = [&](int k0) {
     const bool fullk = (k0 + BK <= K);
-    if (fastA && fullk) {
+    if constexpr (MAP) {
+      if (fastA && fullk) {
+#pragma unroll
+        for (int r = 0; r < VA; r++) va[r] = *reinterpret_cast<const d2_t *>(pA + (size_t)amap[k0 + a_kc + r * (512 / BM)] * lda);
+      } else {
+#pragma unroll
+        for (int r = 0; r < VA; r++) {
+          const int gm0 = bm + 2 * a_mv, gk = k0 + a_kc + r * (512 / BM);
+          d2_t v = (d2_t){0.0, 0.0};
+          if (gk < K) {
+            const double *col = A + (size_t)amap[gk] * lda;
+            if (gm0 < M) v.x = col[gm0];
+            if (gm0 + 1 < M) v.y = col[gm0 + 1];
+          }
+          va[r] = v;
+        }
+      }
+    } else if (fastA && fullk) {
       if (!transA) {
 #pragma unroll
         for (int r = 0; r < VA; r++) va[r] = *reinterpret_cast<const d2_t *>(pA + (size_t)(k0 + r * (512 / BM)) * lda);
@@ -256,7 +274,9 @@
       for (int r = 0; r < 4; r++) {
         int gm = bm + wm + i * 16 + l15, gn = bn + wn + j * 16 + l4 + 4 * r;
         if (gm < M && gn < N) {
-          size_t o = (size_t)gn * ldc + gm;
+          size_t o;
+          if constexpr (MAP) o = (size_t)cmap[gn] * ldc + gm;
+          else o = (size_t)gn * ldc + gm;
           double v = alpha * acc(i, j, r);
           if (splitk) {
             unsafeAtomicAdd(&C[o], v);
@@ -289,6 +309,18 @@
   if ((int)blockIdx.x >= nt) return;
   dgemm_tile<BM, BN, ACC, MF>(blockIdx.x, t.tA, t.tB, t.M, t.N, t.K, t.alpha, t.A, t.lda, t.B, t.ldb, t.beta, t.C, t.ldc,
                               As, Bs, sym, 0, -1, t.over);
+}
+
+template <int MF = 1>
+__global__ __launch_bounds__(256, 2) void k_dgemm_tasklist_map(const GemmTask *__restrict__ tasks) {
+  __shared__ __attribute__((aligned(16))) double As[2][16][64 + 16];
+  __shared__ __attribute__((aligned(16))) double Bs[2][16][64 + 16];
+  const GemmTask t = tasks[blockIdx.y];
+  if (t.M <= 0 || t.N <= 0) return;
+  const int nt = ((t.M + 63) / 64) * ((t.N + 63) / 64);
+  if ((int)blockIdx.x >= nt) return;
+  dgemm_tile<64, 64, false, MF, true>(blockIdx.x, 0, 0, t.M, t.N, t.K, t.alpha, t.A, t.lda, t.B, t.ldb, 0.0, t.C, t.ldc, As, Bs, 0,
+                                      0, -1, 0, t.amap, t.cmap);
 }
 
 template <int BM, int BN, bool SPLIT = false>
@@ -385,6 +417,15 @@
   HFG_HIP_CHECK(hipGetLastError());
 }
 
+void gemm_tasklist64_map_dev(hfg_ctx *ctx, const GemmTask *dtasks, int ntasks, int maxM, int maxN) {
+  if (ntasks <= 0 || maxM <= 0 || maxN <= 0) return;
+  ProfScope ps(ctx, "gemm");
+  const int tiles = ((maxM + 63) / 64) * ((maxN + 63) / 64);
+  if (mfma4()) hipLaunchKernelGGL((k_dgemm_tasklist_map<0>), dim3(tiles, ntasks), dim3(256), 0, ctx->stream, dtasks);
+  else hipLaunchKernelGGL((k_dgemm_tasklist_map<1>), dim3(tiles, ntasks), dim3(256), 0, ctx->stream, dtasks);
+  HFG_HIP_CHECK(hipGetLastError());
+}
+
 void gemm_tasklist_rect_dev(hfg_ctx *ctx, const GemmTask *dtasks, int ntasks, int maxM, int maxN) {
   if (ntasks <= 0 || maxM <= 0 || maxN <= 0) return;
   ProfScope ps(ctx, "gemm");
diff --git a/helfem_amd/csrc/host/tuning.h b/helfem_amd/csrc/host/tuning.h
--- a/helfem_amd/csrc/host/tuning.h
+++ b/helfem_amd/csrc/host/tuning.h
@@ -42,6 +42,7 @@
   X(trdf_c, int, -1, "HELFEM_TRDF_C", false, "int", atoi(e), "measurement replay of k_trdf only: column-in-panel index forced for every launch (negative: each launch's own)") \
   X(tridiag_ql, bool, false, "HELFEM_TRIDIAG", false, "=ql", !strcmp(e, "ql"), "one-lane implicit QL for the tridiagonal problem instead of divide and conquer (checker)") \
   X(dc_gemm_small, bool, false, "HELFEM_DC_GEMM", false, "=small", !strcmp(e, "small"), "Q U of the divide-and-conquer merges by the first 64 x 64 kernel instead of the tile engine (checker)") \
+  X(dc_levels, bool, false, "HELFEM_DC", false, "=levels", !strcmp(e, "levels"), "divide-and-conquer merges with the gather, scatter and copy-back passes over Q and ten launches per level (checker of the column-mapped product)") \
   X(dc_dbg, bool, false, "HELFEM_DC_DBG", false, "present", true, "merge statistics of divide and conquer on stderr") \
   X(bt_column, bool, false, "HELFEM_BT", false, "=column", !strcmp(e, "column"), "back-transformation reflector by reflector instead of compact WY (checker)") \
   X(bt_fold, bool, true, "HELFEM_BT_FOLD", false, "off if 0", atoi(e) != 0, "X Q formed on the side stream beside divide and conquer; off: Z <- Q Z on the main stream behind it") \
```

Result: faster. 8.520 ms, median of 6 (-1.9%).
